# Spockuto/drand

Measured on AMD Instinct MI355X. Metric: beacons verified/s (batch chain verify), higher is better.
Workload: dtype u32 (381-bit Montgomery, 12x32-bit limbs); 1 GPU; configs[1]: 1000000-round chained beacon history per GPU, chain.VerifyBeacon per round; beacons_per_gpu=1000000, segment_len=64, parallelism=range-shard x1

## Files before the change

drand_amd/_lib.py:

```python
from __future__ import annotations

import ctypes
import os

_HERE = os.path.dirname(os.path.abspath(__file__))
LIB_PATH = os.environ.get("DRAND_AMD_LIB", os.path.join(_HERE, "libblsverify.so"))

BLSV_OK = 0
BLSV_EINVAL = -1
BLSV_EHIP = -2
BLSV_ENOGROUP = -3
BLSV_ENOTENOUGH = -4

AGG_OK = 0
AGG_OK_V2 = 1
AGG_V1_RECOVER_FAIL = 2
AGG_V1_INVALID = 3
AGG_V2_RECOVER_FAIL = 4

REJ_OK = 0
REJ_LENGTH = 1
REJ_FLAG = 2
REJ_INF_NONZERO = 3
REJ_X_GE_P = 4
REJ_NOT_ON_CURVE = 5
REJ_NOT_IN_SUBGROUP = 6
REJ_PAIRING = 7
REJ_SHARE_INDEX = 8

REJ_NAMES = {
    REJ_OK: "ok",
    REJ_LENGTH: "bad length",
    REJ_FLAG: "bad compression flag",
    REJ_INF_NONZERO: "infinity with non-zero bits",
    REJ_X_GE_P: "coordinate >= p",
    REJ_NOT_ON_CURVE: "point is not on curve",
    REJ_NOT_IN_SUBGROUP: "point is not on correct subgroup",
    REJ_PAIRING: "bls: invalid signature",
    REJ_SHARE_INDEX: "tbls: invalid signature share",
}

u8p = ctypes.POINTER(ctypes.c_uint8)
u32p = ctypes.POINTER(ctypes.c_uint32)
u64p = ctypes.POINTER(ctypes.c_uint64)
vp = ctypes.c_void_p
sz = ctypes.c_size_t

SIGNATURES = {
    "blsv_version": (ctypes.c_char_p, []),
    "blsv_device_count": (ctypes.c_int, []),
    "blsv_create": (ctypes.c_int, [ctypes.c_int, ctypes.POINTER(vp)]),
    "blsv_destroy": (None, [vp]),
    "blsv_last_error": (ctypes.c_char_p, [vp]),
    "blsv_synchronize": (ctypes.c_int, [vp]),
    "blsv_set_group": (ctypes.c_int, [vp, u8p, sz, sz]),
    "blsv_verify_chained": (ctypes.c_int, [vp, ctypes.c_uint64, u8p, sz, u8p, sz, u8p, u64p, u8p]),
    "blsv_verify_chained_multi": (ctypes.c_int, [ctypes.POINTER(vp), sz, ctypes.POINTER(sz), ctypes.c_uint64, u8p, sz,
                                                  u8p, sz, u8p, u64p, u8p]),
    "blsv_verify_prevs": (ctypes.c_int, [vp, ctypes.c_uint64, u8p, sz, u8p, sz, u8p, u64p, u8p]),
    "blsv_verify_unchained": (ctypes.c_int, [vp, u64p, ctypes.c_uint64, u8p, sz, u8p, u64p, u8p]),
    "blsv_verify_messages": (ctypes.c_int, [vp, u8p, u8p, u32p, sz, u8p, u8p, u64p, u8p]),
    "blsv_verify_partials": (ctypes.c_int, [vp, u8p, sz, u8p, sz, sz, u8p, u8p]),
    "blsv_verify_partials_multi": (ctypes.c_int, [vp, u8p, u32p, u8p, sz, sz, u8p, u8p]),
    "blsv_recover": (ctypes.c_int, [vp, u8p, sz, u8p, sz, sz, sz, sz, u8p]),
    "blsv_aggregate": (ctypes.c_int, [vp, u8p, sz, u8p, sz, sz, sz, sz, u8p, u8p, u8p, u8p]),
    "blsv_aggregate_round": (ctypes.c_int, [vp, u8p, sz, u8p, sz, u8p, sz, u8p, sz, sz, sz, sz, u8p, u8p, u8p, u8p,
                                             ctypes.POINTER(ctypes.c_int32), u8p]),
    "blsv_sign": (ctypes.c_int, [vp, u8p, ctypes.c_int32, u8p, u32p, sz, u8p]),
    "blsv_verify_chained_dev": (ctypes.c_int, [vp, ctypes.c_uint64, ctypes.c_uint64, ctypes.c_uint64, vp, sz, vp, sz,
                                                vp, vp, vp, vp]),
    "blsv_generate_chained_dev": (ctypes.c_int, [vp, u8p, ctypes.c_uint64, ctypes.c_uint64, vp, sz, vp, sz, vp]),
    "blsv_profile_enable": (ctypes.c_int, [vp, ctypes.c_int]),
    "blsv_profile_read": (ctypes.c_int, [vp, ctypes.POINTER(ctypes.c_double), u64p, u64p, ctypes.c_int]),
    "blsv_lat_trace": (ctypes.c_int, [vp, u64p, ctypes.c_int, ctypes.POINTER(ctypes.c_double), ctypes.c_int]),
    "blsv_test_fp_mul": (ctypes.c_int, [vp, u32p, u32p, sz, u32p]),
    "blsv_test_op": (ctypes.c_int, [vp, ctypes.c_char_p, u32p, sz, u32p]),
    "blsv_test_op_info": (ctypes.c_int, [ctypes.c_int, ctypes.POINTER(ctypes.c_char_p), ctypes.POINTER(ctypes.c_int),
                                         ctypes.POINTER(ctypes.c_int), ctypes.POINTER(ctypes.c_int)]),
    "blsv_test_pairing": (ctypes.c_int, [vp, u32p, u32p, sz, u32p]),
    "blsv_test_hash_to_g2": (ctypes.c_int, [vp, u8p, u32p, sz, u32p, u8p]),
    "blsv_test_final_exp": (ctypes.c_int, [vp, u32p, sz, u32p, u32p]),
    "blsv_set_lat_max": (sz, [vp, sz]),
    "blsv_set_chunk": (sz, [vp, sz]),
    "blsv_workspace_bytes": (sz, [vp]),
    "blsv_lat_trace_enable": (ctypes.c_int, [vp, ctypes.c_int]),
    "blsv_test_generic_chains": (ctypes.c_int, [vp, ctypes.c_int]),
    "blsv_test_spec_stats": (ctypes.c_int, [vp, ctypes.POINTER(ctypes.c_uint64), ctypes.POINTER(ctypes.c_uint64)]),
    "blsv_test_lagrange": (ctypes.c_int, [ctypes.POINTER(ctypes.c_uint32), ctypes.c_size_t, ctypes.POINTER(ctypes.c_uint32)]),
    "blsv_service_create": (ctypes.c_int, [ctypes.c_int, ctypes.c_uint32, ctypes.c_uint32, ctypes.POINTER(vp)]),
    "blsv_service_destroy": (None, [vp]),
    "blsv_service_verify_partial": (ctypes.c_int, [vp, u8p, sz, sz, u8p, sz, u8p, sz, u8p, u8p]),
    "blsv_service_verify_recovered": (ctypes.c_int, [vp, u8p, u8p, sz, u8p, u8p, u8p]),
    "blsv_service_stats": (ctypes.c_int, [vp, u64p, u64p, u64p]),
    "blsv_test_service_limits": (ctypes.c_int, [vp, sz, sz, sz, u64p]),
    "blsv_verify_chained_rlc": (ctypes.c_int, [vp, ctypes.c_uint64, u8p, sz, u8p, sz, u8p, u64p, u8p]),
    "blsv_verify_unchained_rlc": (ctypes.c_int, [vp, u64p, ctypes.c_uint64, u8p, sz, u8p, u64p, u8p]),
    "blsv_verify_chained_rlc_dev": (ctypes.c_int, [vp, ctypes.c_uint64, ctypes.c_uint64, ctypes.c_uint64, vp, sz, vp,
                                                    sz, vp, vp, vp, vp]),
    "blsv_set_rlc_group": (sz, [vp, sz]),
    "blsv_rlc_stats": (ctypes.c_int, [vp, u64p, u64p, u64p]),
    "blsv_test_rlc_seed": (ctypes.c_int, [vp, u8p]),
    "blsv_test_rlc_sums": (ctypes.c_int, [vp, ctypes.c_uint64, u8p, sz, u8p, sz, u8p, u8p]),
    "blsv_tlock_open": (ctypes.c_int, [vp, u8p, u8p, sz, u8p, u8p, u8p, u8p]),
    "blsv_tlock_open_dev": (ctypes.c_int, [vp, u8p, vp, sz, vp, vp, vp]),
    "blsv_tlock_stats": (ctypes.c_int, [vp, u64p, u64p]),
}

_lib = None


class EngineUnavailable(RuntimeError):
    """The HIP engine library could not be loaded (no silent fallback exists)."""


def load():
    global _lib
    if _lib is not None:
        return _lib
    if not os.path.exists(LIB_PATH):
        raise EngineUnavailable(
            f"{LIB_PATH} not found: build it with `python -c 'import __graft_entry__ as g; g.build()'` "
            "(make -C drand_amd/csrc); drand_amd has no CPU fallback")
    try:
        lib = ctypes.CDLL(LIB_PATH)
    except OSError as e:
        raise EngineUnavailable(f"cannot load {LIB_PATH}: {e}") from e
    for name, (res, args) in SIGNATURES.items():
        fn = getattr(lib, name)
        fn.restype = res
        fn.argtypes = args
    _lib = lib
    return lib


def buf(data):
    if data is None:
        return None
    b = bytes(data)
    arr = (ctypes.c_uint8 * max(len(b), 1)).from_buffer_copy(b if b else b"\0")
    return arr


def out_buf(n):
    return (ctypes.c_uint8 * max(n, 1))()
```

drand_amd/csrc/blsverify.cpp:

```cpp
#include "host_internal.h"

void release_workspace(blsv_ctx* c) {
  for (DBuf* d : {&c->H, &c->HQ, &c->S, &c->F, &c->FW, &c->LN, &c->h_inf, &c->s_inf, &c->cls}) d->release();
  c->cap = 0;
}

int ensure_workspace(blsv_ctx* c, size_t cnt) {
  for (;;) {
    size_t want = std::min(std::max(cnt, size_t(64)), c->chunk);
    want = (want + 63) & ~size_t(63);
    if (want <= c->cap) return BLSV_OK;
    hipError_t e = hipSuccess;
    auto need = [&](DBuf& d, size_t bytes) {
      if (e == hipSuccess) e = d.ensure(bytes);
    };
    need(c->H, want * blsk::H_WORDS * 4);
    need(c->HQ, want * blsk::HQ_WORDS * 4);
    need(c->S, want * blsk::S_WORDS * 4);
    need(c->F, want * blsk::F_WORDS * 4);
    need(c->FW, 3 * want * blsk::F_WORDS * 4);
    need(c->LN, std::max(std::min(want, kLineSub) * blsk::MILLER_LINE_WORDS, blsk::FEXP_PARK_WORDS(want)) * 4);
    need(c->h_inf, want);
    need(c->s_inf, want);
    need(c->cls, want);
    static_assert(3 * blsk::F_WORDS >= 48 * 64 / 21 + 1, "FW holds the Miller park of a sub-chunk");
    if (e == hipSuccess) {
      c->cap = want;
      return BLSV_OK;
    }
    release_workspace(c);
    (void)hipGetLastError();
    if (e != hipErrorOutOfMemory || want <= kMinChunk)
      return fail(c, BLSV_EHIP, "staging for %zu items: %s", want, hipGetErrorString(e));
    c->chunk = std::max(kMinChunk, ((want / 2) + 63) & ~size_t(63));
    c->lat_max = std::min(c->lat_max, c->chunk);
    c->oom_halvings++;
  }
}

hipError_t h2d(blsv_ctx* c, void* dst, const void* src, size_t len) {
  if (!len) return hipSuccess;
  if (len > kIoCap / 4) return hipMemcpyAsync(dst, src, len, hipMemcpyHostToDevice, c->stream);
  if (!c->io_up.p) {
    hipError_t e = c->io_up.ensure(kIoCap);
    if (e != hipSuccess) return e;
  }
  if (c->io_up_off + len > kIoCap) {
    hipError_t e = hipStreamSynchronize(c->stream);
    if (e != hipSuccess) return e;
    c->io_up_off = 0;
  }
  uint8_t* h = c->io_up.as<uint8_t>() + c->io_up_off;
  memcpy(h, src, len);
  c->io_up_off += (len + 63) & ~size_t(63);
  return hipMemcpyAsync(dst, h, len, hipMemcpyHostToDevice, c->stream);
}

hipError_t download_sync(blsv_ctx* c, std::initializer_list<Down> ds) {
  size_t total = 0;
  for (const Down& d : ds) total += (d.len + 63) & ~size_t(63);
  const bool staged = total <= kIoCap && (c->io_down.p || c->io_down.ensure(kIoCap) == hipSuccess);
  hipError_t e = hipSuccess;
  size_t off = 0;
  for (const Down& d : ds) {
    if (!d.len) continue;
    void* to = staged ? (void*)(c->io_down.as<uint8_t>() + off) : d.user;
    if (e == hipSuccess) e = hipMemcpyAsync(to, d.dev, d.len, hipMemcpyDeviceToHost, c->stream);
    off += (d.len + 63) & ~size_t(63);
  }
  const hipError_t es = hipStreamSynchronize(c->stream);
  if (e == hipSuccess) e = es;
  if (e == hipSuccess) c->io_up_off = 0;
  if (e != hipSuccess || !staged) return e;
  off = 0;
  for (const Down& d : ds) {
    if (d.len) memcpy(d.user, c->io_down.as<uint8_t>() + off, d.len);
    off += (d.len + 63) & ~size_t(63);
  }
  return hipSuccess;
}

hipEvent_t take_event(blsv_ctx* c) {
  if (!c->event_pool.empty()) {
    hipEvent_t e = c->event_pool.back();
    c->event_pool.pop_back();
    return e;
  }
  hipEvent_t e = nullptr;
  if (hipEventCreate(&e) != hipSuccess) return nullptr;
  return e;
}

extern "C" {

const char* blsv_version(void) { return "drand_amd blsverify 0.1 (gfx950)"; }

int blsv_device_count(void) {
  int n = 0;
  return hipGetDeviceCount(&n) == hipSuccess ? n : 0;
}

int blsv_create(int device, blsv_ctx** out) {
  if (!out) return BLSV_EINVAL;
  *out = nullptr;
  blsv_ctx* c = new blsv_ctx();
  c->device = device;
  hipError_t e = hipSetDevice(device);
  if (e == hipSuccess) e = hipStreamCreateWithFlags(&c->stream, hipStreamNonBlocking);
  if (e == hipSuccess) e = hipStreamCreateWithFlags(&c->side, hipStreamNonBlocking);
  if (e == hipSuccess) e = hipStreamCreateWithFlags(&c->side2, hipStreamNonBlocking);
  for (hipEvent_t& ev : c->hash_ev)
    if (e == hipSuccess) e = hipEventCreateWithFlags(&ev, hipEventDisableTiming);
  if (e == hipSuccess) e = hipEventCreateWithFlags(&c->fork_ev, hipEventDisableTiming);
  if (e == hipSuccess) e = hipEventCreateWithFlags(&c->join_ev, hipEventDisableTiming);
  if (e != hipSuccess) {
    fprintf(stderr, "blsv_create: %s\n", hipGetErrorString(e));
    blsv_destroy(c);
    return BLSV_EHIP;
  }
  *out = c;
  return BLSV_OK;
}

void blsv_destroy(blsv_ctx* c) {
  if (!c) return;
  (void)hipSetDevice(c->device);
  for (hipStream_t s : {c->stream, c->side, c->side2}) {
    if (!s) continue;
    (void)hipStreamSynchronize(s);
    (void)hipStreamDestroy(s);
  }
  for (hipEvent_t ev : c->hash_ev)
    if (ev) (void)hipEventDestroy(ev);
  if (c->fork_ev) (void)hipEventDestroy(c->fork_ev);
  if (c->join_ev) (void)hipEventDestroy(c->join_ev);
  (void)hipDeviceSynchronize();
  for (auto& r : c->recs) {
    (void)hipEventDestroy(r.a);
    (void)hipEventDestroy(r.b);
  }
  for (auto e : c->event_pool) (void)hipEventDestroy(e);
  delete c;
}

const char* blsv_last_error(const blsv_ctx* c) { return c ? c->err.c_str() : "null context"; }

int blsv_synchronize(blsv_ctx* c) {
  if (!c) return BLSV_EINVAL;
  HIPCHK(c, hipStreamSynchronize(c->stream));
  return BLSV_OK;
}

int blsv_profile_enable(blsv_ctx* c, int on) {
  if (!c) return BLSV_EINVAL;
  c->prof = on != 0;
  return BLSV_OK;
}

int blsv_profile_read(blsv_ctx* c, double* ms, uint64_t* launches, uint64_t* items, int nstages) {
  if (!c || nstages < 0) return BLSV_EINVAL;
  (void)hipSetDevice(c->device);
  for (int s = 0; s < nstages; s++) {
    if (ms) ms[s] = 0;
    if (launches) launches[s] = 0;
    if (items) items[s] = 0;
  }
  for (auto& r : c->recs) {
    HIPCHK(c, hipEventSynchronize(r.b));
    float t = 0;
    HIPCHK(c, hipEventElapsedTime(&t, r.a, r.b));
    if (r.stage < nstages) {
      if (ms) ms[r.stage] += t;
      if (launches) launches[r.stage] += 1;
      if (items) items[r.stage] += r.items;
    }
    c->event_pool.push_back(r.a);
    c->event_pool.push_back(r.b);
  }
  c->recs.clear();
  return ST_N;
}

size_t blsv_set_lat_max(blsv_ctx* c, size_t lat_max) {
  if (!c) return 0;
  const size_t prev = c->lat_max;
  c->lat_max = std::min(lat_max, c->chunk);
  return prev;
}

size_t blsv_set_chunk(blsv_ctx* c, size_t items) {
  if (!c) return 0;
  const size_t prev = c->chunk;
  size_t v = items ? std::min(std::max(items, kMinChunk), kMaxChunk) : chunk_env();
  v = (v + 63) & ~size_t(63);
  (void)hipSetDevice(c->device);
  if (v < c->cap) {
    (void)hipStreamSynchronize(c->stream);
    (void)hipStreamSynchronize(c->side);
    release_workspace(c);
  }
  c->chunk = v;
  c->lat_max = std::min(c->lat_max, v);
  return prev;
}

size_t blsv_workspace_bytes(const blsv_ctx* c) {
  if (!c) return 0;
  size_t b = 0;
  for (const DBuf* d : {&c->H, &c->HQ, &c->S, &c->F, &c->FW, &c->LN, &c->h_inf, &c->s_inf, &c->cls}) b += d->sz;
  return b;
}

}
```

drand_amd/csrc/engine_ctx.h:

```cpp
#pragma once
#include <hip/hip_runtime.h>

#include <algorithm>
#include <cerrno>
#include <cstdarg>
#include <cstdio>
#include <cstdlib>
#include <cstring>
#include <string>
#include <vector>

#include "../../include/blsverify.h"
#include "kernels.h"

namespace blsv_detail {

constexpr size_t kMaxChunk = size_t(1) << 20;
constexpr size_t kMinChunk = size_t(1) << 14;
constexpr size_t kLineSub = kMaxChunk;
constexpr size_t kPkTable = 4096;
constexpr size_t kStagingBytesPerItem =
    4 * (blsk::H_WORDS + blsk::HQ_WORDS + blsk::S_WORDS + 4 * blsk::F_WORDS + blsk::MILLER_LINE_WORDS) + 3;
static_assert(576ull * kMaxChunk < 0x7fffffffull, "SoA object resource exceeds its 31-bit num_records");
static_assert((133ull * kMaxChunk) * 4 < 0xffffffffull, "SoA VGPR byte offset exceeds 32 bits");
static_assert(48ull * 4 * kMaxChunk < 0x7fffffffull, "3-lane park slot resource exceeds 31 bits");
static_assert(blsk::G1_WORDS <= blsk::H_WORDS, "timelock: the U table does not fit the H staging");
static_assert(blsk::F_WORDS <= blsk::HQ_WORDS, "timelock: the captured Fp12 does not fit the HQ staging");
static_assert(BLSV_GT_LEN == 4 * blsk::F_WORDS, "timelock: the Gt encoding is one F staging row per item");
static_assert(BLSV_U_LEN <= 4 * blsk::S_WORDS, "timelock: a host call's compressed U bytes do not fit the S staging");

struct DBuf {
  void* p = nullptr;
  size_t sz = 0;
  ~DBuf() {
    if (p) (void)hipFree(p);
  }
  void release() {
    if (p) (void)hipFree(p);
    p = nullptr;
    sz = 0;
  }
  hipError_t ensure(size_t need) {
    if (need <= sz) return hipSuccess;
    if (p) {
      (void)hipFree(p);
      p = nullptr;
      sz = 0;
    }
    size_t want = std::max(need, size_t(256));
    hipError_t e = hipMalloc(&p, want);
    if (e == hipSuccess) sz = want;
    return e;
  }
  template <typename T>
  T* as() const {
    return static_cast<T*>(p);
  }
};

struct PinBuf {
  void* p = nullptr;
  size_t sz = 0;
  ~PinBuf() {
    if (p) (void)hipHostFree(p);
  }
  hipError_t ensure(size_t need) {
    if (need <= sz) return hipSuccess;
    if (p) (void)hipHostFree(p);
    p = nullptr;
    sz = 0;
    const size_t want = std::max(need + need / 2, size_t(4096));
    hipError_t e = hipHostMalloc(&p, want, hipHostMallocDefault);
    if (e == hipSuccess) sz = want;
    return e;
  }
  template <typename T>
  T* as() const {
    return static_cast<T*>(p);
  }
};

}
using namespace blsv_detail;

enum Stage {
  ST_HASH = 0,
  ST_DECOMP = 1,
  ST_MILLER = 2,
  ST_FEXP = 3,
  ST_FINISH = 4,
  ST_LAT = 5,
  ST_RLC = 6,
  ST_TLOCK = 7,
  ST_N = 8
};
struct ProfRec {
  int stage;
  size_t items;
  hipEvent_t a, b;
};

constexpr size_t kRlcGroupDefault = 64;
constexpr size_t kRlcGroupMin = 8, kRlcGroupMax = 4096;
constexpr size_t kLatMaxDefault = 1536;
inline size_t chunk_env() {
  static const size_t v = [] {
    const char* e = getenv("BLSV_CHUNK");
    if (!e) return kMaxChunk;
    char* end = nullptr;
    errno = 0;
    const unsigned long long x = strtoull(e, &end, 10);
    if (end == e || *end != '\0' || errno == ERANGE || e[0] == '-' || x == 0) {
      fprintf(stderr, "blsverify: ignoring BLSV_CHUNK=\"%s\" (not a positive integer); chunk stays %zu\n", e, kMaxChunk);
      return kMaxChunk;
    }
    const size_t c = (size_t)std::min<unsigned long long>(std::max<unsigned long long>(x, kMinChunk), kMaxChunk);
    return (c + 63) & ~size_t(63);
  }();
  return v;
}

inline size_t lat_max_env() {
  static const size_t v = [] {
    const char* e = getenv("BLSV_LAT_MAX");
    if (!e) return kLatMaxDefault;
    char* end = nullptr;
    errno = 0;
    const unsigned long long x = strtoull(e, &end, 10);
    if (end == e || *end != '\0' || errno == ERANGE || e[0] == '-') {
      fprintf(stderr, "blsverify: ignoring BLSV_LAT_MAX=\"%s\" (not a non-negative integer); cutover stays %zu\n", e,
              kLatMaxDefault);
      return kLatMaxDefault;
    }
    return (size_t)std::min<unsigned long long>(x, kMaxChunk);
  }();
  return v;
}

struct rlc_state {
  size_t group = kRlcGroupDefault;
  bool seed_pinned = false;
  uint8_t seed[32] = {0};
  uint64_t groups = 0, groups_failed = 0, items_exact = 0;
  DBuf part, gH, gS, g_hinf, g_sinf, gcls, cH, cS, c_hinf, c_sinf, ccls, fail, out96;
  PinBuf host;
};

struct tlock_state {
  bool valid = false;
  uint8_t sig[96] = {0};
  uint8_t cls = 0;
  uint64_t prepared = 0, items = 0;
  DBuf d_sig, S, s_inf, s_cls, tab;
};

struct blsv_ctx {
  int device = 0;
  bool prof = false;
  size_t chunk = chunk_env();
  size_t lat_max = std::min(lat_max_env(), chunk);
  uint64_t oom_halvings = 0;
  std::vector<ProfRec> recs;
  std::vector<hipEvent_t> event_pool;
  hipStream_t stream = nullptr;
  hipStream_t side = nullptr;
  hipEvent_t fork_ev = nullptr, join_ev = nullptr;
  hipStream_t side2 = nullptr;
  hipEvent_t hash_ev[2] = {nullptr, nullptr};
  std::string err;
  bool has_group = false;
  size_t t = 0, n = 0;
  DBuf commits, commit_inf;
  std::vector<uint8_t> group_bytes;
  DBuf pk_all, pk_all_inf;
  size_t pk_all_n = 0;
  bool pk_all_built = false;
  DBuf pk_tab, pk_inf;
  uint8_t pk_cache[48];
  bool pk_cache_valid = false;
  size_t cap = 0;
  DBuf H, S, F, FW, LN, h_inf, s_inf, cls;
  DBuf HQ;
  DBuf in_sigs, in_msgs, in_off, in_len, in_rounds, seeds, bitmap, first_bad, sk, idx, lambdas, scratch, out,
      pp_tab, pp_inf, sel, g1_cls, misc;
  PinBuf pin;
  PinBuf io_up, io_down;
  size_t io_up_off = 0;
  struct SpecSlot {
    DBuf sig, S, s_inf, cls, sel, lam, scratch, out, vmsg, voff, vlen, vcls;
    DBuf hout, saff;
    PinBuf host;
  } spec[2];
  uint64_t spec_hits = 0, spec_misses = 0;
  DBuf arena;
  rlc_state rlc;
  tlock_state tlock;
};

#define HIPCHK(ctx, expr)                                                             \
  do {                                                                                \
    hipError_t e_ = (expr);                                                           \
    if (e_ != hipSuccess) return fail((ctx), BLSV_EHIP, "%s: %s", #expr, hipGetErrorString(e_)); \
  } while (0)

inline int fail(blsv_ctx* ctx, int code, const char* fmt, ...) {
  char buf[512];
  va_list ap;
  va_start(ap, fmt);
  vsnprintf(buf, sizeof buf, fmt, ap);
  va_end(ap);
  if (ctx) ctx->err = buf;
  return code;
}


int ensure_workspace(blsv_ctx* c, size_t cnt);
void release_workspace(blsv_ctx* c);

int svc_verify_mixed(blsv_ctx* c, size_t n, const uint8_t* msgs, const uint64_t* off, const uint32_t* lens,
                     const uint8_t* sigs96, const uint32_t* idx, const uint32_t* d_tab, const uint8_t* d_tab_inf,
                     uint8_t* cls_out);
```

drand_amd/csrc/host_internal.h:

```cpp
#pragma once
#include <functional>
#include <initializer_list>

#include "engine_ctx.h"
#include "hostlogic.h"

#pragma GCC visibility push(hidden)

constexpr size_t kIoCap = size_t(1) << 20;
hipError_t h2d(blsv_ctx* c, void* dst, const void* src, size_t len);
struct Down {
  void* user;
  const void* dev;
  size_t len;
};
hipError_t download_sync(blsv_ctx* c, std::initializer_list<Down> ds);

hipEvent_t take_event(blsv_ctx* c);
struct StageTimer {
  blsv_ctx* c;
  int stage;
  size_t items;
  hipStream_t st;
  hipEvent_t a = nullptr;
  StageTimer(blsv_ctx* c_, int stage_, size_t items_, hipStream_t st_) : c(c_), stage(stage_), items(items_), st(st_) {
    if (c->prof && (a = take_event(c))) (void)hipEventRecord(a, st);
  }
  ~StageTimer() {
    if (!a) return;
    hipEvent_t b = take_event(c);
    if (!b) return;
    (void)hipEventRecord(b, st);
    c->recs.push_back({stage, items, a, b});
  }
};

struct Staging {
  uint32_t *H, *HQ, *S, *F, *FW, *LN;
  uint8_t *h_inf, *s_inf, *cls;
};
inline Staging staging(const blsv_ctx* c) {
  return {c->H.as<uint32_t>(),    c->HQ.as<uint32_t>(),   c->S.as<uint32_t>(),
          c->F.as<uint32_t>(),    c->FW.as<uint32_t>(),   c->LN.as<uint32_t>(),
          c->h_inf.as<uint8_t>(), c->s_inf.as<uint8_t>(), c->cls.as<uint8_t>()};
}

struct SigSrc {
  const uint8_t* d;
  size_t stride, offset;
};
struct PkSel {
  const uint32_t* tab;
  const uint8_t* inf;
  const uint32_t* idx;
};
inline PkSel group_pk(const blsv_ctx* c) { return {c->commits.as<uint32_t>(), c->commit_inf.as<uint8_t>(), nullptr}; }

inline void hash_chained(blsv_ctx* c, const blsk::ChainedSrc& src, size_t base, size_t cnt, hipStream_t st) {
  const Staging w = staging(c);
  blsk::launch_hash_chained(src, base, cnt, w.H, w.h_inf, w.HQ, st);
}
inline void hash_messages(blsv_ctx* c, const uint8_t* d_msgs, const uint64_t* d_off, const uint32_t* d_len, size_t base,
                          size_t cnt, hipStream_t st) {
  const Staging w = staging(c);
  blsk::launch_hash_messages(d_msgs, d_off + base, d_len + base, cnt, w.H, w.h_inf, w.HQ, st);
}
inline void hash_uploaded(blsv_ctx* c, size_t base, size_t cnt, hipStream_t st) {
  hash_messages(c, c->in_msgs.as<uint8_t>(), c->in_off.as<uint64_t>(), c->in_len.as<uint32_t>(), base, cnt, st);
}
inline void lat_uploaded(blsv_ctx* c, const SigSrc& sig, size_t cnt, const PkSel& pk, uint8_t* cls, uint32_t* S,
                         uint8_t* s_inf, hipStream_t st) {
  blsk::launch_lat_messages(c->in_msgs.as<uint8_t>(), c->in_off.as<uint64_t>(), c->in_len.as<uint32_t>(), sig.d,
                            sig.stride, sig.offset, cnt, pk.tab, pk.inf, pk.idx, cls, S, s_inf, st);
}
inline void final_exp(blsv_ctx* c, size_t cnt, uint8_t* cls, hipStream_t st, uint32_t* out = nullptr) {
  const Staging w = staging(c);
  blsk::launch_final_exp(w.F, w.FW, cnt, cls, st, w.LN, out);
}

inline bool use_lat(const blsv_ctx* c, size_t n) { return n > 0 && n <= std::min(c->lat_max, c->cap); }
inline bool use_rlc(const blsv_ctx* c, size_t n) { return n > c->lat_max && n >= 2 * c->rlc.group; }

template <typename F>
inline int for_each_pass(const blsv_ctx* c, size_t n, F f) {
  for (size_t base = 0; base < n; base += c->cap) {
    const int rc = f(base, std::min(c->cap, n - base));
    if (rc) return rc;
  }
  return BLSV_OK;
}

using HashFn = std::function<void(size_t base, size_t cnt, hipStream_t st)>;
struct Tail {
  bool randomized = false;
  uint32_t seed[8] = {0};
  bool fused_subgroup() const { return !randomized; }
};
struct PassOut {
  uint64_t* bitmap;
  unsigned long long* first_bad;
  uint8_t* cls;
  uint64_t label0;
};
int run_head(blsv_ctx* c, const SigSrc& sig, size_t base, size_t cnt, const Tail& tail, hipStream_t st,
             const HashFn& hash);
int run_passes(blsv_ctx* c, size_t n, const SigSrc& sig, const PkSel& pk, const HashFn& hash, const Tail& tail,
               const PassOut& out, hipStream_t st);
int ctx_outputs(blsv_ctx* c, size_t n, bool with_cls, PassOut& out);

int rlc_draw_seed(blsv_ctx* c, uint32_t (&w)[8]);
int rlc_sums(blsv_ctx* c, size_t base, size_t cnt, const uint32_t (&seed)[8], hipStream_t st);

int stage_chain(blsv_ctx* c, uint64_t first_round, const uint8_t* prevs, size_t prev0_len, bool prev_rows,
                const uint8_t* sigs96, size_t n, blsk::ChainedSrc& src);
int decode_g1(blsv_ctx* c, const uint8_t* pk48, size_t cnt, DBuf& tab, DBuf& inf, std::vector<uint8_t>& cls);
int upload_messages(blsv_ctx* c, const uint8_t* msgs, const uint32_t* msg_lens, size_t n);

#pragma GCC visibility pop
```

drand_amd/csrc/hostlogic.h:

```cpp
#pragma once
#include <stddef.h>
#include <stdint.h>

#include <algorithm>
#include <vector>

#include "../../include/blsverify.h"

#pragma GCC visibility push(hidden)
namespace blsv_detail {

inline void scalar_mod_r(const uint8_t* be32, uint32_t out[8]) {
  static const uint32_t R[8] = {0x00000001u, 0xffffffffu, 0xfffe5bfeu, 0x53bda402u,
                                0x09a1d805u, 0x3339d808u, 0x299d7d48u, 0x73eda753u};
  for (int i = 0; i < 8; i++) {
    const uint8_t* q = be32 + 28 - 4 * i;
    out[i] = ((uint32_t)q[0] << 24) | ((uint32_t)q[1] << 16) | ((uint32_t)q[2] << 8) | q[3];
  }
  for (int rep = 0; rep < 4; rep++) {
    bool ge = true;
    for (int i = 7; i >= 0; i--) {
      if (out[i] != R[i]) {
        ge = out[i] > R[i];
        break;
      }
    }
    if (!ge) break;
    uint64_t br = 0;
    for (int i = 0; i < 8; i++) {
      uint64_t d = (uint64_t)out[i] - R[i] - br;
      out[i] = (uint32_t)d;
      br = (d >> 63) & 1;
    }
  }
}

namespace hfr {
typedef unsigned __int128 u128;
static const uint64_t RM[4] = {0xffffffff00000001ull, 0x53bda402fffe5bfeull, 0x3339d80809a1d805ull,
                               0x73eda753299d7d48ull};
struct E {
  uint64_t l[4];
};
inline bool geq_r(const uint64_t (&a)[5]) {
  if (a[4]) return true;
  for (int i = 3; i >= 0; i--)
    if (a[i] != RM[i]) return a[i] > RM[i];
  return true;
}
inline void sub_r(uint64_t (&a)[5]) {
  uint64_t br = 0;
  for (int i = 0; i < 4; i++) {
    const u128 d = (u128)a[i] - RM[i] - br;
    a[i] = (uint64_t)d;
    br = (uint64_t)(d >> 64) & 1u;
  }
  a[4] -= br;
}
inline uint64_t n0() {
  uint64_t inv = 1;
  for (int k = 0; k < 7; k++) inv *= 2 - RM[0] * inv;
  return (uint64_t)0 - inv;
}
inline E mul(const E& a, const E& b) {
  static const uint64_t N0 = n0();
  uint64_t t[6] = {0, 0, 0, 0, 0, 0};
  for (int i = 0; i < 4; i++) {
    uint64_t c = 0;
    for (int j = 0; j < 4; j++) {
      const u128 v = (u128)a.l[j] * b.l[i] + t[j] + c;
      t[j] = (uint64_t)v;
      c = (uint64_t)(v >> 64);
    }
    u128 v = (u128)t[4] + c;
    t[4] = (uint64_t)v;
    t[5] = (uint64_t)(v >> 64);
    const uint64_t m = t[0] * N0;
    v = (u128)m * RM[0] + t[0];
    c = (uint64_t)(v >> 64);
    for (int j = 1; j < 4; j++) {
      v = (u128)m * RM[j] + t[j] + c;
      t[j - 1] = (uint64_t)v;
      c = (uint64_t)(v >> 64);
    }
    v = (u128)t[4] + c;
    t[3] = (uint64_t)v;
    t[4] = t[5] + (uint64_t)(v >> 64);
  }
  uint64_t r[5] = {t[0], t[1], t[2], t[3], t[4]};
  if (geq_r(r)) sub_r(r);
  return {{r[0], r[1], r[2], r[3]}};
}
inline E add(const E& a, const E& b) {
  uint64_t r[5];
  uint64_t c = 0;
  for (int i = 0; i < 4; i++) {
    const u128 v = (u128)a.l[i] + b.l[i] + c;
    r[i] = (uint64_t)v;
    c = (uint64_t)(v >> 64);
  }
  r[4] = c;
  if (geq_r(r)) sub_r(r);
  return {{r[0], r[1], r[2], r[3]}};
}
inline const E& r2() {
  static const E v = [] {
    E x = {{1, 0, 0, 0}};
    for (int k = 0; k < 512; k++) x = add(x, x);
    return x;
  }();
  return v;
}
inline E from_int(int64_t v) {
  E x = {{(uint64_t)(v < 0 ? -v : v), 0, 0, 0}};
  if (v < 0) {
    uint64_t a[5] = {RM[0], RM[1], RM[2], RM[3], 0};
    uint64_t br = 0;
    for (int i = 0; i < 4; i++) {
      const u128 d = (u128)a[i] - x.l[i] - br;
      a[i] = (uint64_t)d;
      br = (uint64_t)(d >> 64) & 1u;
    }
    x = {{a[0], a[1], a[2], a[3]}};
  }
  return mul(x, r2());
}
inline E inv(const E& a) {
  uint64_t e[4] = {RM[0] - 2, RM[1], RM[2], RM[3]};
  E acc = from_int(1);
  for (int i = 255; i >= 0; i--) {
    acc = mul(acc, acc);
    if ((e[i >> 6] >> (i & 63)) & 1u) acc = mul(acc, a);
  }
  return acc;
}
}

inline void host_lagrange(const uint32_t* idx, size_t t, uint32_t* out) {
  std::vector<hfr::E> num(t), den(t), pre(t + 1);
  for (size_t i = 0; i < t; i++) {
    const int64_t xi = (int64_t)idx[i] + 1;
    hfr::E n = hfr::from_int(1), d = n;
    for (size_t j = 0; j < t; j++) {
      if (j == i) continue;
      const int64_t xj = (int64_t)idx[j] + 1;
      n = hfr::mul(n, hfr::from_int(xj));
      d = hfr::mul(d, hfr::from_int(xj - xi));
    }
    num[i] = n;
    den[i] = d;
  }
  pre[0] = hfr::from_int(1);
  for (size_t i = 0; i < t; i++) pre[i + 1] = hfr::mul(pre[i], den[i]);
  hfr::E run = hfr::inv(pre[t]);
  const hfr::E one_plain = {{1, 0, 0, 0}};
  for (size_t i = t; i-- > 0;) {
    const hfr::E di = hfr::mul(run, pre[i]);
    run = hfr::mul(run, den[i]);
    const hfr::E lam = hfr::mul(hfr::mul(num[i], di), one_plain);
    for (int w = 0; w < 4; w++) {
      out[i * 8 + 2 * w] = (uint32_t)lam.l[w];
      out[i * 8 + 2 * w + 1] = (uint32_t)(lam.l[w] >> 32);
    }
  }
}

inline void bitmap_words_to_bytes(const uint64_t* w, size_t n, uint8_t* out) {
  for (size_t i = 0; i < (n + 7) / 8; i++) {
    uint8_t b = (uint8_t)(w[i / 8] >> (8 * (i % 8)));
    if (i == (n + 7) / 8 - 1 && (n % 8)) b &= (uint8_t)((1u << (n % 8)) - 1);
    out[i] = b;
  }
}

inline uint64_t fold_classes(const uint8_t* cls, size_t n, uint8_t* ok_bitmap) {
  uint64_t fb = UINT64_MAX;
  for (size_t i = 0; i < n; i++) {
    if (cls[i] != BLSV_REJ_OK && fb == UINT64_MAX) fb = i;
    if (ok_bitmap) {
      if (i % 8 == 0) ok_bitmap[i / 8] = 0;
      ok_bitmap[i / 8] |= (uint8_t)((cls[i] == BLSV_REJ_OK) << (i % 8));
    }
  }
  return fb;
}

inline void or_bits_at(uint8_t* dst, const uint8_t* src, size_t cnt, size_t pos) {
  const size_t nb = (cnt + 7) / 8, q = pos / 8, s = pos % 8;
  for (size_t j = 0; j < nb; j++) {
    uint8_t b = src[j];
    if (j == nb - 1 && (cnt % 8)) b &= (uint8_t)((1u << (cnt % 8)) - 1);
    dst[q + j] |= (uint8_t)(b << s);
    if (s && (b >> (8 - s))) dst[q + j + 1] |= (uint8_t)(b >> (8 - s));
  }
}

inline void share_indices(const uint8_t* partials, size_t partial_len, size_t k, std::vector<uint32_t>& index) {
  index.assign(k, 0);
  if (partial_len < 2) return;
  for (size_t i = 0; i < k; i++) index[i] = ((uint32_t)partials[i * partial_len] << 8) | partials[i * partial_len + 1];
}

inline bool select_shares(const std::vector<uint8_t>& cls, const std::vector<uint32_t>& index, size_t lo, size_t hi,
                          size_t t, size_t n, std::vector<uint32_t>& sel, std::vector<uint32_t>& idx) {
  sel.clear();
  idx.clear();
  size_t taken = 0;
  for (size_t i = lo; i < hi && taken < t; i++) {
    if (cls[i] != BLSV_REJ_OK) continue;
    taken++;
    if (index[i] >= n || std::find(idx.begin(), idx.end(), index[i]) != idx.end()) continue;
    sel.push_back((uint32_t)i);
    idx.push_back(index[i]);
  }
  return sel.size() >= t;
}

inline size_t rlc_failing_items(size_t cnt, size_t G, const uint32_t* fail, size_t nf) {
  const size_t ng = (cnt + G - 1) / G;
  return nf * G - (fail[nf - 1] == ng - 1 ? ng * G - cnt : 0);
}

struct SvcLayout {
  size_t o_len, o_idx, o_sig, o_msg, total;
};
inline SvcLayout svc_layout(size_t n, size_t mbytes) {
  SvcLayout l;
  l.o_len = (n + 1) * 8;
  l.o_idx = l.o_len + ((n * 4 + 7) & ~size_t(7));
  l.o_sig = l.o_idx + ((n * 4 + 7) & ~size_t(7));
  l.o_msg = l.o_sig + n * 96;
  l.total = l.o_msg + mbytes + 8;
  return l;
}

}
#pragma GCC visibility pop
```

drand_amd/csrc/k_fexp.hip:

```cpp
#include "kcommon.h"

namespace blsk {

BLS_KERNEL(BLS_WPE_FEXP) k_fexp_easy(const uint32_t* F, size_t cnt, const uint8_t* cls, uint32_t* G) {
  size_t i = (size_t)blockIdx.x * TPB + threadIdx.x;
  if (i >= cnt || cls[i] != REJ_OK) return;
  st_fp12(G, cnt, i, fexp_easy(ld_fp12(F, cnt, i)));
}

#ifndef BLS_WPE_FEXP_TRI
#define BLS_WPE_FEXP_TRI 2
#endif

struct TriPark {
  uint32_t* p;
  size_t n, i;
};

template <typename LoadX>
DI fp4 tri_pow_x_abs(const tri_lane& t, LoadX lx, const TriPark& pk) {
  constexpr uint64_t NSQ = 1ull | (2ull << 6) | (3ull << 12) | (9ull << 18) | (32ull << 24) | (16ull << 30);
  fp4 r = lx();
#pragma unroll 1
  for (int s = 0; s < 6; s++) {
    const int n = (int)((NSQ >> (6 * s)) & 63u);
#pragma unroll 1
    for (int k = 0; k < n; k++) r = tri_cyclotomic_sqr(t, r);
    if (s < 5) r = tri_mul_lp(t, r, lx(), pk.p, pk.n, pk.i);
  }
  return r;
}

template <int MODE>
BLS_KERNEL(BLS_WPE_FEXP_TRI) k_fexp_tri(const uint32_t* X, const uint32_t* C, const uint32_t* G, size_t cnt,
                                        uint8_t* cls, uint32_t* OUT, uint32_t* park) {
  const tri_lane t = tri_lane_id();
#if BLS_CSQR_LIN
  kp_lds_init<11>();
#endif
  const size_t ir = (size_t)blockIdx.x * TRI_GROUPS + t.group;
  const bool in_range = t.group < TRI_GROUPS && ir < cnt;
  const size_t i0 = in_range ? ir : cnt - 1;
  const bool live = in_range && cls[i0] == REJ_OK;
  const TriPark pk = {park, (size_t)gridDim.x * TPB, (size_t)blockIdx.x * TPB + t.lane};
  auto at = [&](const uint32_t* B) {
    size_t j = i0;
    asm volatile("" : "+v"(j));
    return tri_load(B, cnt, j, t.role);
  };
  fp4 r = tri_conj(t, tri_pow_x_abs(t, [&]() { return at(X); }, pk));
  if (MODE == 0 || MODE == 1) r = tri_mul_lp(t, r, tri_conj(t, at(X)), pk.p, pk.n, pk.i);
  if (MODE == 2) r = tri_mul_lp(t, r, tri_frob(t, at(X)), pk.p, pk.n, pk.i);
  if (MODE == 4) {
    r = tri_mul_lp(t, r, tri_frob2(t, at(C)), pk.p, pk.n, pk.i);
    r = tri_mul_lp(t, r, tri_conj(t, at(C)), pk.p, pk.n, pk.i);
    r = tri_mul_lp(t, r, tri_cyclotomic_sqr(t, at(G)), pk.p, pk.n, pk.i);
    r = tri_mul_lp(t, r, at(G), pk.p, pk.n, pk.i);
  }
  if (MODE < 4 || OUT) {
    if (live) tri_store(OUT, cnt, i0, t.role, r);
  }
  if (MODE == 4) {
    const bool one = tri_is_one(t, r);
    if (live && t.role == 0 && !one) cls[i0] = REJ_PAIRING;
  }
}

void launch_final_exp(uint32_t* F, uint32_t* W, size_t cnt, uint8_t* cls, hipStream_t st, uint32_t* park,
                      uint32_t* out) {
  if (!cnt) return;
  uint32_t* G = W;
  uint32_t* B = W + cnt * F_WORDS;
  uint32_t* C = W + 2 * cnt * F_WORDS;
  const dim3 grid(grid_for(cnt)), blk(TPB);
  hipLaunchKernelGGL(k_fexp_easy, grid, blk, 0, st, F, cnt, cls, G);
  const dim3 tgrid((unsigned)((cnt + TRI_GROUPS - 1) / TRI_GROUPS));
  hipLaunchKernelGGL(k_fexp_tri<0>, tgrid, blk, 0, st, G, nullptr, nullptr, cnt, cls, F, park);
  hipLaunchKernelGGL(k_fexp_tri<1>, tgrid, blk, 0, st, F, nullptr, nullptr, cnt, cls, B, park);
  hipLaunchKernelGGL(k_fexp_tri<2>, tgrid, blk, 0, st, B, nullptr, nullptr, cnt, cls, C, park);
  hipLaunchKernelGGL(k_fexp_tri<3>, tgrid, blk, 0, st, C, nullptr, nullptr, cnt, cls, F, park);
  hipLaunchKernelGGL(k_fexp_tri<4>, tgrid, blk, 0, st, F, C, G, cnt, cls, out, park);
}

}
```

drand_amd/csrc/k_miller.hip:

```cpp
#include <type_traits>

#include "kcommon.h"
#include "testops.h"

namespace blsk {

DI int line_slot(int step, int k) { return (step * 2 + k) * 6; }
#ifndef BLS_LN_AUX
#define BLS_LN_AUX 2
#endif
#ifndef BLS_LN_AUX_ST
#define BLS_LN_AUX_ST BLS_LN_AUX
#endif
#ifndef BLS_LN_AUX_LD
#define BLS_LN_AUX_LD BLS_LN_AUX
#endif

static __shared__ uint32_t g_ml_T[72 * BLS_LANES];
struct g2proj_lds {
  uint32_t* base;
  DI fp2 get(int c) const {
    fp2 v;
#pragma unroll
    for (int w = 0; w < 12; w++) {
      v.c0.l[w] = base[(24 * c + w) * BLS_LANES];
      v.c1.l[w] = base[(24 * c + 12 + w) * BLS_LANES];
    }
    return v;
  }
  DI void set(int c, const fp2& v) const {
#pragma unroll
    for (int w = 0; w < 12; w++) {
      base[(24 * c + w) * BLS_LANES] = v.c0.l[w];
      base[(24 * c + 12 + w) * BLS_LANES] = v.c1.l[w];
    }
  }
};

template <bool CHECK>
BLS_KERNEL(BLS_WPE_LINES)
k_miller_lines(const uint32_t* pk_tab, const uint8_t* pk_inf, const uint32_t* pk_idx, const uint32_t* H,
               const uint8_t* h_inf, const uint32_t* S, const uint8_t* s_inf,
               std::conditional_t<CHECK, uint8_t*, const uint8_t*> cls, size_t cnt, size_t base, size_t m, size_t sub,
               uint32_t* LN) {
  const int k = (int)(blockIdx.x & 1u);
  const size_t i = (size_t)(blockIdx.x >> 1) * TPB + threadIdx.x;
  if (i >= m) return;
  const size_t g = base + i;
  if (cls[g] != REJ_OK) return;
  const uint32_t kk = pk_idx ? pk_idx[g] : 0u;
  const bool act[2] = {!(pk_inf[kk] | h_inf[g]), !s_inf[g]};
  {
    const uint32_t* Qb = k == 0 ? H : S;
    auto load_q = [&]() {
      size_t j = g;
      asm volatile("" : "+v"(j));
      return g2a{ld_fp2(Qb, cnt, j, 0), ld_fp2(Qb, cnt, j, 2)};
    };
    auto emit = [&](int step, const line& l) {
      const int s = line_slot(step, k);
      const line o = act[k] ? l : line_one();
      st_fp2<BLS_LN_AUX_ST>(LN, sub, i, s + 0, o.a0);
      st_fp2<BLS_LN_AUX_ST>(LN, sub, i, s + 2, o.a1);
      st_fp2<BLS_LN_AUX_ST>(LN, sub, i, s + 4, o.a4);
    };
    auto pcoord = [&](int c) {
      size_t o = (size_t)kk * G1_WORDS + 12 * c;
      asm volatile("" : "+v"(o));
      fp v;
#pragma unroll
      for (int w = 0; w < 12; w++) v.l[w] = pk_tab[o + w];
      return k == 0 ? v : fp_load_const(c == 0 ? G1_GEN_X : G1_GEN_NEG_Y);
    };
    if (!act[k]) {
#pragma unroll 1
      for (int s = 0; s < MILLER_STEPS; s++) emit(s, line_one());
      return;
    }
    int step = 0;
    auto put = [&](int c, const fp2& v) { st_fp2<BLS_LN_AUX_ST>(LN, sub, i, line_slot(step, k) + 2 * c, v); };
    auto xp = [&]() { return pcoord(0); };
    auto yp = [&]() { return pcoord(1); };
    const g2proj_lds T{g_ml_T + threadIdx.x};
    {
      const g2a Q0 = load_q();
      T.set(0, Q0.x);
      T.set(1, Q0.y);
      T.set(2, fp2_one());
    }
#pragma unroll 1
    for (int b = 62; b >= 0; b--) {
      miller_dbl_step_ts(T, put, xp, yp);
      step++;
      if ((BLS_X_ABS >> b) & 1ull) {
        miller_add_step_ts(T, load_q, put, xp, yp);
        step++;
      }
    }
    if constexpr (CHECK) {
      if (k == 1 && !miller_t_in_subgroup(T, load_q)) {
        size_t j = g;
        asm volatile("" : "+v"(j));
        cls[j] = REJ_NOT_IN_SUBGROUP;
      }
    }
  }
}

static __shared__ uint32_t g_mf_L[120 * BLS_LANES];
DI void mf_put(int c, const fp2& v) {
  const unsigned l = threadIdx.x;
#pragma unroll
  for (int k = 0; k < 12; k++) {
    g_mf_L[(c * 24 + k) * BLS_LANES + l] = v.c0.l[k];
    g_mf_L[(c * 24 + 12 + k) * BLS_LANES + l] = v.c1.l[k];
  }
}
DI fp2 mf_get(int c) {
  unsigned l = threadIdx.x;
  asm volatile("" : "+v"(l));
  fp2 v;
#pragma unroll
  for (int k = 0; k < 12; k++) {
    v.c0.l[k] = g_mf_L[(c * 24 + k) * BLS_LANES + l];
    v.c1.l[k] = g_mf_L[(c * 24 + 12 + k) * BLS_LANES + l];
  }
  return v;
}
using KpLds16 = KpLdsK<16>;

template <typename LB>
DI fp6 fp6_mul_lb(const fp6& a, LB lb) {
#if BLS_F6_LIN
  return fp6_mul_lin_lb(a, lb, KpLds16());
#else
  fp2 t0 = fp2_mul(a.c0, lb(0));
  fp2 t1 = fp2_mul(a.c1, lb(1));
  fp2 t2 = fp2_mul(a.c2, lb(2));
  fp2 c0 = fp2_add(fp2_mul_xi(fp2_sub(fp2_sub(fp2_mul(fp2_add_lazy(a.c1, a.c2), fp2_add_lazy(lb(1), lb(2))), t1), t2)), t0);
  fp2 c1 = fp2_add(fp2_sub(fp2_sub(fp2_mul(fp2_add_lazy(a.c0, a.c1), fp2_add_lazy(lb(0), lb(1))), t0), t1), fp2_mul_xi(t2));
  fp2 c2 = fp2_add(fp2_sub(fp2_sub(fp2_mul(fp2_add_lazy(a.c0, a.c2), fp2_add_lazy(lb(0), lb(2))), t0), t2), t1);
  return {c0, c1, c2};
#endif
}
DI fp12 fp12_mul_by_line_pair_lds(const fp12& f) {
  const fp6 t0 = fp6_mul_lb(f.c0, [](int c) { return mf_get(c); });
  fp6 t1;
  {
    const fp2 b1 = mf_get(3), b2 = mf_get(4);
    t1 = fp6_mul_by_12(f.c1, b1, b2);
  }
  const fp6 c1 = fp6_sub(fp6_sub(fp6_mul_lb(fp6_add_lazy(f.c0, f.c1), [](int c) {
                                   return c == 0 ? mf_get(0) : fp2_add_lazy(mf_get(c), mf_get(c + 2));
                                 }),
                                 t0),
                         t1);
  return {fp6_add(t0, fp6_mul_v(t1)), c1};
}

BLS_KERNEL(BLS_WPE_MILLER_F) k_miller_f(const uint32_t* LN, const uint8_t* cls, size_t cnt, size_t base,
                                                  size_t m, size_t sub, uint32_t* F) {
#if BLS_F6_LIN
  kp_lds_init<16>();
#endif
  const size_t i = (size_t)blockIdx.x * TPB + threadIdx.x;
  if (i >= m) return;
  const size_t g = base + i;
  if (cls[g] != REJ_OK) return;
  auto load = [&](int step, int k) {
    const int s = line_slot(step, k);
    return line{ld_fp2<BLS_LN_AUX_LD>(LN, sub, i, s + 0), ld_fp2<BLS_LN_AUX_LD>(LN, sub, i, s + 2),
                ld_fp2<BLS_LN_AUX_LD>(LN, sub, i, s + 4)};
  };
  fp12 f = fp12_one();
  int step = 0;
#pragma unroll 1
  for (int b = 62; b >= 0; b--) {
#pragma unroll 1
    for (int rep = 0; rep < 2; rep++) {
      if (rep == 1 && !((BLS_X_ABS >> b) & 1ull)) break;
#if BLS_F6_LIN
      if (rep == 0 && b != 62) f = fp12_sqr_lin(f, KpLds16());
#else
      if (rep == 0 && b != 62) f = fp12_sqr(f);
#endif
      {
        const fp12 L = line_mul_line(load(step, 0), load(step, 1));
        if (step == 0) {
          f = L;
          step++;
          continue;
        }
        mf_put(0, L.c0.c0);
        mf_put(1, L.c0.c1);
        mf_put(2, L.c0.c2);
        mf_put(3, L.c1.c1);
        mf_put(4, L.c1.c2);
      }
      f = fp12_mul_by_line_pair_lds(f);
      step++;
    }
  }
  st_fp12(F, cnt, g, fp12_conj(f));
}

constexpr uint64_t miller_sq_bits(int half) {
  uint64_t m = 0;
  int s = 0;
  for (int i = 62; i >= 0; i--) {
    if (i != 62 && s / 64 == half) m |= 1ull << (s % 64);
    s++;
    if ((BLS_X_ABS >> i) & 1ull) s++;
  }
  return m;
}
constexpr uint64_t MILLER_SQ_LO = miller_sq_bits(0), MILLER_SQ_HI = miller_sq_bits(1);

#ifndef BLS_MILLER_TRI_MAX
#define BLS_MILLER_TRI_MAX 65536
#endif
constexpr size_t kMillerTriMax = BLS_MILLER_TRI_MAX;

#ifndef BLS_WPE_MILLER_TRI
#define BLS_WPE_MILLER_TRI 2
#endif

BLS_KERNEL(BLS_WPE_MILLER_TRI) k_miller_f_tri(const uint32_t* LN, const uint8_t* cls, size_t cnt, size_t base,
                                              size_t m, size_t sub, uint32_t* F, uint32_t* park) {
  const tri_lane t = tri_lane_id();
  const size_t ir = (size_t)blockIdx.x * TRI_GROUPS + t.group;
  const bool in_range = t.group < TRI_GROUPS && ir < m;
  const size_t i = in_range ? ir : m - 1;
  const bool live = in_range && cls[base + i] == REJ_OK;
  const size_t park_n = (size_t)gridDim.x * TPB, park_i = (size_t)blockIdx.x * TPB + t.lane;
  fp4 A;
#pragma unroll 1
  for (int s = 0; s < MILLER_STEPS; s++) {
    const bool sq = ((s < 64 ? MILLER_SQ_LO >> s : MILLER_SQ_HI >> (s - 64)) & 1ull) != 0;
    if (sq) A = tri_sqr_lp(t, A);
    const int s0 = line_slot(s, 0), s1 = line_slot(s, 1);
    auto la = [&](int c) {
      size_t j = i;
      asm volatile("" : "+v"(j));
      return ld_fp2_v<BLS_LN_AUX_LD>(LN + (size_t)s0 * 12 * sub, sub, j, 2 * c);
    };
    auto lb = [&](int c) {
      size_t j = i;
      asm volatile("" : "+v"(j));
      return ld_fp2_v<BLS_LN_AUX_LD>(LN + (size_t)s1 * 12 * sub, sub, j, 2 * c);
    };
    const fp4 L = tri_line_pair(t, la, lb);
    if (s == 0) {
      A = L;
    } else {
      A = tri_mul_lp(t, A, L, park, park_n, park_i);
    }
  }
  A = tri_conj(t, A);
  if (live) tri_store(F, cnt, base + i, t.role, A);
}

template <int OP, int NIN, int NOUT>
__global__ void __launch_bounds__(TPB) k_test_op_mf(const uint32_t* in, size_t cnt, uint32_t* out) {
#if BLS_F6_LIN
  kp_lds_init<16>();
#endif
  const size_t i = (size_t)blockIdx.x * TPB + threadIdx.x;
  if (i >= cnt) return;
  fp x[NIN], r[NOUT];
#pragma unroll
  for (int k = 0; k < NIN; k++)
#pragma unroll
    for (int w = 0; w < 12; w++) x[k].l[w] = in[(i * NIN + k) * 12 + w];
  if constexpr (OP == TOP_fp6_mul_lb) {
#pragma unroll
    for (int c = 0; c < 3; c++) mf_put(c, t_f2(x, 6 + 2 * c));
    t_put6(r, 0, fp6_mul_lb(t_f6(x, 0), [](int c) { return mf_get(c); }));
  } else {
#pragma unroll
    for (int c = 0; c < 5; c++) mf_put(c, t_f2(x, 12 + 2 * c));
    t_put12(r, 0, fp12_mul_by_line_pair_lds(t_f12(x, 0)));
  }
#pragma unroll
  for (int k = 0; k < NOUT; k++)
#pragma unroll
    for (int w = 0; w < 12; w++) out[(i * NOUT + k) * 12 + w] = r[k].l[w];
}

bool launch_test_op_mf(int op, const uint32_t* in, size_t cnt, uint32_t* out, hipStream_t st) {
  if (op != TOP_fp6_mul_lb && op != TOP_fp12_mul_by_line_pair_lds) return false;
  if (!cnt) return true;
  if (op == TOP_fp6_mul_lb)
    hipLaunchKernelGGL((k_test_op_mf<TOP_fp6_mul_lb, 12, 6>), dim3(grid_for(cnt)), dim3(TPB), 0, st, in, cnt, out);
  else
    hipLaunchKernelGGL((k_test_op_mf<TOP_fp12_mul_by_line_pair_lds, 22, 12>), dim3(grid_for(cnt)), dim3(TPB), 0, st, in,
                       cnt, out);
  return true;
}

void launch_miller(const uint32_t* pk_tab, const uint8_t* pk_inf, const uint32_t* pk_idx, const uint32_t* H,
                   const uint8_t* h_inf, const uint32_t* S, const uint8_t* s_inf, uint8_t* cls, size_t cnt,
                   uint32_t* F, uint32_t* LN, size_t sub, uint32_t* park, bool check_subgroup, hipStream_t st) {
  if (!cnt) return;
  for (size_t b = 0; b < cnt; b += sub) {
    const size_t m = cnt - b < sub ? cnt - b : sub;
    if (check_subgroup)
      hipLaunchKernelGGL(k_miller_lines<true>, dim3(2 * grid_for(m)), dim3(TPB), 0, st, pk_tab, pk_inf, pk_idx, H,
                         h_inf, S, s_inf, cls, cnt, b, m, sub, LN);
    else
      hipLaunchKernelGGL(k_miller_lines<false>, dim3(2 * grid_for(m)), dim3(TPB), 0, st, pk_tab, pk_inf, pk_idx, H,
                         h_inf, S, s_inf, (const uint8_t*)cls, cnt, b, m, sub, LN);
    if (m <= kMillerTriMax) {
      hipLaunchKernelGGL(k_miller_f_tri, dim3((unsigned)((m + TRI_GROUPS - 1) / TRI_GROUPS)), dim3(TPB), 0, st, LN,
                         cls, cnt, b, m, sub, F, park);
    } else {
      hipLaunchKernelGGL(k_miller_f, dim3(grid_for(m)), dim3(TPB), 0, st, LN, cls, cnt, b, m, sub, F);
    }
  }
}

}
```

drand_amd/csrc/kernels.h:

```cpp
#pragma once
#include <hip/hip_runtime.h>
#include <stddef.h>
#include <stdint.h>

namespace blsk {

constexpr int H_WORDS = 48;
constexpr int S_WORDS = 48;
constexpr int F_WORDS = 144;
constexpr int G1_WORDS = 24;

struct ChainedSrc {
  const uint8_t* sigs;
  const uint8_t* seeds;
  uint64_t first_round;
  uint64_t seg_len;
  uint32_t seed0_len;
  uint64_t seg_phase;
};

constexpr int HQ_WORDS = 144;
void launch_hash_chained(const ChainedSrc& src, size_t base, size_t cnt, uint32_t* H, uint8_t* h_inf,
                         uint32_t* Q, hipStream_t st);
void launch_hash_unchained(const uint64_t* rounds, uint64_t first_round, size_t base, size_t cnt, uint32_t* H,
                           uint8_t* h_inf, uint32_t* Q, hipStream_t st);
void launch_hash_messages(const uint8_t* msgs, const uint64_t* off, const uint32_t* len, size_t cnt,
                          uint32_t* H, uint8_t* h_inf, uint32_t* Q, hipStream_t st);
void launch_decompress_g2(const uint8_t* sigs, size_t stride, size_t offset, size_t base, size_t cnt, uint32_t* S,
                          uint8_t* s_inf, uint8_t* cls, hipStream_t st);
constexpr int MILLER_LINE_WORDS = 68 * 2 * 6 * 12;
void launch_miller(const uint32_t* pk_tab, const uint8_t* pk_inf, const uint32_t* pk_idx, const uint32_t* H,
                   const uint8_t* h_inf, const uint32_t* S, const uint8_t* s_inf, uint8_t* cls, size_t cnt,
                   uint32_t* F, uint32_t* LN, size_t sub, uint32_t* park, bool check_subgroup, hipStream_t st);
constexpr size_t TRI_PARK_WORDS(size_t items) { return 48 * 64 * ((items + 20) / 21); }
constexpr size_t FEXP_PARK_WORDS(size_t items) { return TRI_PARK_WORDS(items); }
void launch_final_exp(uint32_t* F, uint32_t* W, size_t cnt, uint8_t* cls, hipStream_t st, uint32_t* park,
                      uint32_t* out = nullptr);
void launch_finish(const uint8_t* cls, size_t base, size_t cnt, uint64_t* bitmap, unsigned long long* first_bad,
                   uint64_t label0, hipStream_t st);

constexpr size_t kRlcLaneItems = 8;
constexpr size_t kRlcPartWords = 72;
constexpr size_t rlc_lanes(size_t cnt) { return (cnt + kRlcLaneItems - 1) / kRlcLaneItems; }
constexpr size_t rlc_groups(size_t cnt, size_t group) { return (cnt + group - 1) / group; }
void launch_rlc_sums(const uint32_t* H, const uint8_t* h_inf, const uint32_t* S, const uint8_t* s_inf,
                     const uint8_t* cls, size_t cnt, uint64_t index0, const uint32_t* seed_words, size_t group,
                     uint32_t* part, uint32_t* GH, uint8_t* g_hinf, uint32_t* GS, uint8_t* g_sinf, hipStream_t st);
void launch_rlc_gather(const uint32_t* fail, size_t group, size_t m, const uint32_t* H, const uint8_t* h_inf,
                       const uint32_t* S, const uint8_t* s_inf, const uint8_t* cls, size_t cnt, uint32_t* CH,
                       uint8_t* c_hinf, uint32_t* CS, uint8_t* c_sinf, uint8_t* ccls, hipStream_t st);
void launch_rlc_scatter(const uint32_t* fail, size_t group, size_t m, const uint8_t* ccls, uint8_t* cls, size_t cnt,
                        hipStream_t st);
void launch_rlc_compress(const uint32_t* GP, const uint8_t* g_inf, size_t ng, uint8_t* out96, hipStream_t st);

constexpr size_t kTlockTabWords = 68 * 3 * 24;
void launch_tlock_prepare(const uint32_t* S, const uint8_t* s_inf, const uint8_t* s_cls, uint32_t* tab, hipStream_t st);
void launch_tlock_f(const uint32_t* tab, const uint32_t* U, const uint8_t* u_inf, const uint8_t* cls,
                    const uint8_t* sig_inf, size_t cnt, uint32_t* F, hipStream_t st);
void launch_tlock_encode(const uint32_t* E, const uint8_t* cls, size_t cnt, uint8_t* out, hipStream_t st);

int lat_trace_read(uint64_t* out, int n, hipStream_t st);
int lat_trace_clear(hipStream_t st);
int lat_trace_enable(int on, hipStream_t st);
extern int g_generic_chains_all;
void launch_lat_chained(const ChainedSrc& src, size_t base, size_t cnt, const uint32_t* pk_tab, const uint8_t* pk_inf,
                        uint8_t* cls, hipStream_t st);
void launch_lat_unchained(const uint64_t* rounds, uint64_t first_round, const uint8_t* sigs, size_t base, size_t cnt,
                          const uint32_t* pk_tab, const uint8_t* pk_inf, uint8_t* cls, hipStream_t st);
void launch_lat_messages(const uint8_t* msgs, const uint64_t* off, const uint32_t* len, const uint8_t* sigs,
                         size_t stride, size_t offset, size_t cnt, const uint32_t* pk_tab, const uint8_t* pk_inf,
                         const uint32_t* pk_idx, uint8_t* cls, uint32_t* S, uint8_t* s_inf, hipStream_t st);

void launch_decompress_g1(const uint8_t* in, size_t cnt, uint32_t* tab, uint8_t* inf, uint8_t* cls, hipStream_t st);
void launch_pubpoly_eval(const uint32_t* commits, const uint8_t* commit_inf, uint32_t t, const uint32_t* idx,
                         size_t cnt, uint32_t* out_tab, uint8_t* out_inf, hipStream_t st);
void launch_lat_decode(const uint8_t* sigs, size_t stride, size_t offset, size_t cnt, uint32_t* S, uint8_t* s_inf,
                       uint8_t* cls, hipStream_t st);
void launch_decompress_g2_only(const uint8_t* sigs, size_t stride, size_t offset, size_t base, size_t cnt,
                               uint32_t* S, uint8_t* s_inf, uint8_t* cls, hipStream_t st);
void launch_lat_recover(const uint32_t* S, size_t n_s, const uint8_t* s_inf, const uint32_t* sel,
                        const uint32_t* lambdas, uint32_t t, uint32_t* scratch, uint8_t* out96, hipStream_t st,
                        uint32_t* saff = nullptr);
constexpr size_t kLatHoutWords = 448, kLatSaffWords = 192;
void launch_lat_hash_key(const uint8_t* msgs, const uint64_t* off, const uint32_t* len, const uint32_t* pk_tab,
                         const uint8_t* pk_inf, uint32_t* hout, hipStream_t st);
void launch_lat_verify_pre(const uint32_t* hout, const uint32_t* saff, uint8_t* cls, hipStream_t st);
void launch_sign(const uint32_t* sk_words, int32_t index, const uint32_t* H, const uint8_t* h_inf, size_t cnt,
                 uint8_t* out, size_t out_stride, hipStream_t st);
void launch_gen_chained(const uint32_t* sk_words, const ChainedSrc& src, size_t n, uint8_t* sigs_out, hipStream_t st);

bool launch_test_op(int op, const uint32_t* in, size_t cnt, uint32_t* out, uint32_t* park, hipStream_t st);
bool launch_test_op_mf(int op, const uint32_t* in, size_t cnt, uint32_t* out, hipStream_t st);
void launch_test_fp_mul(const uint32_t* a, const uint32_t* b, size_t cnt, uint32_t* out, hipStream_t st);
void launch_test_pairing(const uint32_t* p_tab, const uint32_t* q_aff, size_t cnt, uint32_t* out_f, hipStream_t st);
void launch_test_unpack_g2(const uint32_t* H, size_t cnt, uint32_t* out, hipStream_t st);
void launch_test_pack_fp12(const uint32_t* f, size_t cnt, uint32_t* F, hipStream_t st);
void launch_test_unpack_fp12(const uint32_t* F, size_t cnt, uint32_t* out, hipStream_t st);
void launch_test_final_exp_ref(const uint32_t* F, size_t cnt, uint32_t* out, hipStream_t st);

}
```

drand_amd/csrc/testhooks.cpp:

```cpp
#include "../../include/blsverify_testing.h"
#include "host_internal.h"
#include "testops_list.h"

static const bls::TestOpInfo* find_test_op(const char* name, int* op) {
  if (!name) return nullptr;
  const bls::TestOpInfo* tab = bls::test_op_table();
  for (int k = 0; k < bls::TOP_COUNT; k++)
    if (!strcmp(tab[k].name, name)) {
      if (op) *op = k;
      return &tab[k];
    }
  return nullptr;
}

extern "C" {

int blsv_test_lagrange(const uint32_t* idx, size_t t, uint32_t* out) {
  if (!idx || !out) return BLSV_EINVAL;
  for (size_t i = 0; i < t; i++)
    for (size_t j = 0; j < i; j++)
      if (idx[i] == idx[j]) return BLSV_EINVAL;
  host_lagrange(idx, t, out);
  return BLSV_OK;
}

int blsv_test_rlc_seed(blsv_ctx* c, const uint8_t* seed32) {
  if (!c) return BLSV_EINVAL;
  c->rlc.seed_pinned = seed32 != nullptr;
  if (seed32) memcpy(c->rlc.seed, seed32, 32);
  return BLSV_OK;
}

int blsv_test_rlc_sums(blsv_ctx* c, uint64_t first_round, const uint8_t* prev0, size_t prev0_len,
                       const uint8_t* sigs96, size_t n, uint8_t* out_a96, uint8_t* out_b96) {
  if (!c) return BLSV_EINVAL;
  if (!n || !sigs96 || !prev0 || !out_a96 || !out_b96 || (prev0_len != 32 && prev0_len != 96))
    return fail(c, BLSV_EINVAL, "test_rlc_sums: bad arguments");
  (void)hipSetDevice(c->device);
  Tail tail;
  tail.randomized = true;
  int rc = rlc_draw_seed(c, tail.seed);
  if (rc) return rc;
  rc = ensure_workspace(c, n);
  if (rc) return rc;
  blsk::ChainedSrc src;
  rc = stage_chain(c, first_round, prev0, prev0_len, false, sigs96, n, src);
  if (rc) return rc;
  rlc_state& r = c->rlc;
  size_t done = 0;
  rc = for_each_pass(c, n, [&](size_t base, size_t cnt) {
    const size_t ng = blsk::rlc_groups(cnt, r.group);
    int prc = run_head(c, {src.sigs, 96, 0}, base, cnt, tail, c->stream,
                       [&](size_t b, size_t m, hipStream_t st) { hash_chained(c, src, b, m, st); });
    if (prc) return prc;
    prc = rlc_sums(c, base, cnt, tail.seed, c->stream);
    if (prc) return prc;
    HIPCHK(c, r.out96.ensure(2 * ng * 96));
    uint8_t* d_out = r.out96.as<uint8_t>();
    blsk::launch_rlc_compress(r.gH.as<uint32_t>(), r.g_hinf.as<uint8_t>(), ng, d_out, c->stream);
    blsk::launch_rlc_compress(r.gS.as<uint32_t>(), r.g_sinf.as<uint8_t>(), ng, d_out + ng * 96, c->stream);
    HIPCHK(c, hipGetLastError());
    HIPCHK(c, hipMemcpyAsync(out_a96 + done * 96, d_out, ng * 96, hipMemcpyDeviceToHost, c->stream));
    HIPCHK(c, hipMemcpyAsync(out_b96 + done * 96, d_out + ng * 96, ng * 96, hipMemcpyDeviceToHost, c->stream));
    HIPCHK(c, hipStreamSynchronize(c->stream));
    c->io_up_off = 0;
    done += ng;
    return BLSV_OK;
  });
  return rc ? rc : (int)done;
}

int blsv_test_spec_stats(blsv_ctx* c, uint64_t* hits, uint64_t* misses) {
  if (!c || !hits || !misses) return BLSV_EINVAL;
  *hits = c->spec_hits;
  *misses = c->spec_misses;
  return BLSV_OK;
}

int blsv_test_generic_chains(blsv_ctx* c, int on) {
  if (!c) return BLSV_EINVAL;
  blsk::g_generic_chains_all = on != 0;
  return BLSV_OK;
}

int blsv_lat_trace_enable(blsv_ctx* c, int on) {
  if (!c) return BLSV_EINVAL;
  (void)hipSetDevice(c->device);
  if (blsk::lat_trace_enable(on, c->stream) != 0) return fail(c, BLSV_EHIP, "lat_trace_enable: symbol copy failed");
  return BLSV_OK;
}

int blsv_lat_trace(blsv_ctx* c, uint64_t* ticks, int n, double* ticks_per_us, int clear) {
  if (!c || n < 0 || (n && !ticks)) return BLSV_EINVAL;
  (void)hipSetDevice(c->device);
  HIPCHK(c, hipDeviceSynchronize());
  int got = 0;
  if (n) {
    got = blsk::lat_trace_read(ticks, n, c->stream);
    if (got < 0) return fail(c, BLSV_EHIP, "lat_trace: symbol copy failed");
  }
  if (ticks_per_us) {
    int khz = 0;
    HIPCHK(c, hipDeviceGetAttribute(&khz, hipDeviceAttributeWallClockRate, c->device));
    *ticks_per_us = khz / 1000.0;
  }
  if (clear && blsk::lat_trace_clear(c->stream) != 0) return fail(c, BLSV_EHIP, "lat_trace: clear failed");
  HIPCHK(c, hipStreamSynchronize(c->stream));
  return got;
}

int blsv_test_fp_mul(blsv_ctx* c, const uint32_t* a, const uint32_t* b, size_t n, uint32_t* out) {
  if (!c || (n && (!a || !b || !out))) return BLSV_EINVAL;
  (void)hipSetDevice(c->device);
  DBuf da, db, dout;
  HIPCHK(c, da.ensure(n * 48));
  HIPCHK(c, db.ensure(n * 48));
  HIPCHK(c, dout.ensure(n * 48));
  HIPCHK(c, hipMemcpyAsync(da.p, a, n * 48, hipMemcpyHostToDevice, c->stream));
  HIPCHK(c, hipMemcpyAsync(db.p, b, n * 48, hipMemcpyHostToDevice, c->stream));
  blsk::launch_test_fp_mul(da.as<uint32_t>(), db.as<uint32_t>(), n, dout.as<uint32_t>(), c->stream);
  HIPCHK(c, hipGetLastError());
  HIPCHK(c, hipMemcpyAsync(out, dout.p, n * 48, hipMemcpyDeviceToHost, c->stream));
  HIPCHK(c, hipStreamSynchronize(c->stream));
  return BLSV_OK;
}

int blsv_test_pairing(blsv_ctx* c, const uint32_t* p, const uint32_t* q, size_t n, uint32_t* out_f) {
  if (!c || (n && (!p || !q || !out_f))) return BLSV_EINVAL;
  (void)hipSetDevice(c->device);
  DBuf dp, dq, dout;
  HIPCHK(c, dp.ensure(n * 96));
  HIPCHK(c, dq.ensure(n * 192));
  HIPCHK(c, dout.ensure(n * 576));
  HIPCHK(c, hipMemcpyAsync(dp.p, p, n * 96, hipMemcpyHostToDevice, c->stream));
  HIPCHK(c, hipMemcpyAsync(dq.p, q, n * 192, hipMemcpyHostToDevice, c->stream));
  blsk::launch_test_pairing(dp.as<uint32_t>(), dq.as<uint32_t>(), n, dout.as<uint32_t>(), c->stream);
  HIPCHK(c, hipGetLastError());
  HIPCHK(c, hipMemcpyAsync(out_f, dout.p, n * 576, hipMemcpyDeviceToHost, c->stream));
  HIPCHK(c, hipStreamSynchronize(c->stream));
  return BLSV_OK;
}

int blsv_test_final_exp(blsv_ctx* c, const uint32_t* f, size_t n, uint32_t* out_pipeline, uint32_t* out_ref) {
  if (!c || (n && (!f || !out_pipeline || !out_ref))) return BLSV_EINVAL;
  if (n > kMaxChunk) return BLSV_EINVAL;
  (void)hipSetDevice(c->device);
  int rc = ensure_workspace(c, n);
  if (rc) return rc;
  if (n > c->cap) return fail(c, BLSV_EINVAL, "test_final_exp: more than the context chunk");
  if (!n) return BLSV_OK;
  DBuf din, dout, dref;
  HIPCHK(c, din.ensure(n * 576));
  HIPCHK(c, dout.ensure(n * 576));
  HIPCHK(c, dref.ensure(n * 576));
  const Staging w = staging(c);
  HIPCHK(c, hipMemcpyAsync(din.p, f, n * 576, hipMemcpyHostToDevice, c->stream));
  HIPCHK(c, hipMemsetAsync(w.cls, 0, n, c->stream));
  blsk::launch_test_pack_fp12(din.as<uint32_t>(), n, w.F, c->stream);
  blsk::launch_test_final_exp_ref(w.F, n, dref.as<uint32_t>(), c->stream);
  final_exp(c, n, w.cls, c->stream, dout.as<uint32_t>());
  blsk::launch_test_unpack_fp12(dout.as<uint32_t>(), n, din.as<uint32_t>(), c->stream);
  HIPCHK(c, hipMemcpyAsync(out_pipeline, din.p, n * 576, hipMemcpyDeviceToHost, c->stream));
  blsk::launch_test_unpack_fp12(dref.as<uint32_t>(), n, dout.as<uint32_t>(), c->stream);
  HIPCHK(c, hipMemcpyAsync(out_ref, dout.p, n * 576, hipMemcpyDeviceToHost, c->stream));
  HIPCHK(c, hipGetLastError());
  HIPCHK(c, hipStreamSynchronize(c->stream));
  return BLSV_OK;
}

int blsv_test_op_info(int index, const char** name, int* in_fp, int* out_fp, int* lanes) {
  if (index < 0 || index >= bls::TOP_COUNT) return BLSV_EINVAL;
  const bls::TestOpInfo& t = bls::test_op_table()[index];
  if (name) *name = t.name;
  if (in_fp) *in_fp = t.nin;
  if (out_fp) *out_fp = t.nout;
  if (lanes) *lanes = t.kind == 3 ? 3 : 1;
  return BLSV_OK;
}

int blsv_test_op(blsv_ctx* c, const char* name, const uint32_t* in, size_t n, uint32_t* out) {
  int op = 0;
  const bls::TestOpInfo* t = find_test_op(name, &op);
  if (!c || !t || (n && (!in || !out))) return BLSV_EINVAL;
  if (n > kMaxChunk) return BLSV_EINVAL;
  if (!n) return BLSV_OK;
  (void)hipSetDevice(c->device);
  const size_t in_bytes = n * (size_t)t->nin * 48, out_bytes = n * (size_t)t->nout * 48;
  DBuf din, dout, dpark;
  HIPCHK(c, din.ensure(in_bytes));
  HIPCHK(c, dout.ensure(out_bytes));
  if (t->kind == 3) HIPCHK(c, dpark.ensure(blsk::TRI_PARK_WORDS(n) * 4));
  HIPCHK(c, hipMemcpyAsync(din.p, in, in_bytes, hipMemcpyHostToDevice, c->stream));
  HIPCHK(c, hipMemsetAsync(dout.p, 0xA5, out_bytes, c->stream));
  const bool ran = t->kind == 2
                       ? blsk::launch_test_op_mf(op, din.as<uint32_t>(), n, dout.as<uint32_t>(), c->stream)
                       : blsk::launch_test_op(op, din.as<uint32_t>(), n, dout.as<uint32_t>(),
                                              t->kind == 3 ? dpark.as<uint32_t>() : nullptr, c->stream);
  if (!ran) return fail(c, BLSV_EINVAL, "test_op: no kernel for this op");
  HIPCHK(c, hipGetLastError());
  HIPCHK(c, hipMemcpyAsync(out, dout.p, out_bytes, hipMemcpyDeviceToHost, c->stream));
  HIPCHK(c, hipStreamSynchronize(c->stream));
  return BLSV_OK;
}

int blsv_test_hash_to_g2(blsv_ctx* c, const uint8_t* msgs, const uint32_t* msg_lens, size_t n, uint32_t* out,
                         uint8_t* inf) {
  if (!c || (n && (!msg_lens || !out || !inf))) return BLSV_EINVAL;
  if (n > kMaxChunk) return BLSV_EINVAL;
  (void)hipSetDevice(c->device);
  int rc = ensure_workspace(c, n);
  if (rc) return rc;
  if (n > c->cap) return fail(c, BLSV_EINVAL, "test_hash_to_g2: more than the context chunk");
  rc = upload_messages(c, msgs, msg_lens, n);
  if (rc) return rc;
  DBuf dout;
  HIPCHK(c, dout.ensure(n * 192));
  hash_uploaded(c, 0, n, c->stream);
  blsk::launch_test_unpack_g2(c->H.as<uint32_t>(), n, dout.as<uint32_t>(), c->stream);
  HIPCHK(c, hipGetLastError());
  HIPCHK(c, hipMemcpyAsync(out, dout.p, n * 192, hipMemcpyDeviceToHost, c->stream));
  HIPCHK(c, hipMemcpyAsync(inf, c->h_inf.p, n, hipMemcpyDeviceToHost, c->stream));
  HIPCHK(c, hipStreamSynchronize(c->stream));
  return BLSV_OK;
}

}
```

drand_amd/csrc/tlock.cpp:

```cpp
#include "host_internal.h"

static int tlock_prepare_sig(blsv_ctx* c, const uint8_t* sig96, hipStream_t st, uint8_t* sig_class) {
  tlock_state& t = c->tlock;
  if (!t.valid || memcmp(t.sig, sig96, 96) != 0) {
    t.valid = false;
    HIPCHK(c, t.d_sig.ensure(96));
    HIPCHK(c, t.S.ensure(blsk::S_WORDS * 4));
    HIPCHK(c, t.s_inf.ensure(1));
    HIPCHK(c, t.s_cls.ensure(1));
    HIPCHK(c, t.tab.ensure(blsk::kTlockTabWords * 4));
    HIPCHK(c, hipMemcpyAsync(t.d_sig.p, sig96, 96, hipMemcpyHostToDevice, st));
    {
      StageTimer tm(c, ST_TLOCK, 1, st);
      blsk::launch_decompress_g2(t.d_sig.as<uint8_t>(), 96, 0, 0, 1, t.S.as<uint32_t>(), t.s_inf.as<uint8_t>(),
                                 t.s_cls.as<uint8_t>(), st);
      blsk::launch_tlock_prepare(t.S.as<uint32_t>(), t.s_inf.as<uint8_t>(), t.s_cls.as<uint8_t>(),
                                 t.tab.as<uint32_t>(), st);
    }
    HIPCHK(c, hipGetLastError());
    uint8_t cls = 0xff;
    HIPCHK(c, hipMemcpyAsync(&cls, t.s_cls.p, 1, hipMemcpyDeviceToHost, st));
    HIPCHK(c, hipStreamSynchronize(st));
    memcpy(t.sig, sig96, 96);
    t.cls = cls;
    t.valid = true;
    if (cls == BLSV_REJ_OK) t.prepared++;
  }
  if (sig_class) *sig_class = t.cls;
  if (t.cls != BLSV_REJ_OK) return fail(c, BLSV_EINVAL, "tlock_open: signature rejected (class %d)", (int)t.cls);
  return BLSV_OK;
}

static int tlock_pass(blsv_ctx* c, const uint8_t* d_us, size_t cnt, uint8_t* d_out, uint8_t* d_cls_out,
                      hipStream_t st) {
  const tlock_state& t = c->tlock;
  const Staging w = staging(c);
  uint32_t* U = w.H;
  uint8_t* u_inf = w.h_inf;
  uint8_t* ucls = w.s_inf;
  {
    StageTimer tm(c, ST_DECOMP, cnt, st);
    blsk::launch_decompress_g1(d_us, cnt, U, u_inf, ucls, st);
  }
  HIPCHK(c, hipMemcpyAsync(w.cls, ucls, cnt, hipMemcpyDeviceToDevice, st));
  {
    StageTimer tm(c, ST_TLOCK, cnt, st);
    blsk::launch_tlock_f(t.tab.as<uint32_t>(), U, u_inf, ucls, t.s_inf.as<uint8_t>(), cnt, w.F, st);
  }
  {
    StageTimer tm(c, ST_FEXP, cnt, st);
    final_exp(c, cnt, w.cls, st, w.HQ);
  }
  blsk::launch_tlock_encode(w.HQ, ucls, cnt, d_out, st);
  if (d_cls_out) HIPCHK(c, hipMemcpyAsync(d_cls_out, ucls, cnt, hipMemcpyDeviceToDevice, st));
  HIPCHK(c, hipGetLastError());
  return BLSV_OK;
}

static int tlock_passes(blsv_ctx* c, bool host, const uint8_t* us, size_t n, uint8_t* out, uint8_t* cls,
                        hipStream_t st) {
  int rc = ensure_workspace(c, n);
  if (rc) return rc;
  for (size_t base = 0; base < n; base += c->cap) {
    const size_t cnt = std::min(c->cap, n - base);
    const uint8_t* pass_us = us + base * BLSV_U_LEN;
    uint8_t* pass_out = out + base * BLSV_GT_LEN;
    if (host) {
      HIPCHK(c, h2d(c, c->S.p, pass_us, cnt * BLSV_U_LEN));
      rc = tlock_pass(c, c->S.as<uint8_t>(), cnt, c->F.as<uint8_t>(), nullptr, st);
      if (rc) return rc;
      HIPCHK(c, download_sync(c, {{pass_out, c->F.p, cnt * BLSV_GT_LEN}, {cls + base, c->s_inf.p, cnt}}));
    } else {
      rc = tlock_pass(c, pass_us, cnt, pass_out, cls ? cls + base : nullptr, st);
      if (rc) return rc;
    }
  }
  c->tlock.items += n;
  return BLSV_OK;
}

extern "C" {

int blsv_tlock_open(blsv_ctx* c, const uint8_t* sig96, const uint8_t* us48, size_t n, uint8_t* out_gt576, uint8_t* ok,
                    uint8_t* reject_class, uint8_t* sig_class) {
  if (!c) return BLSV_EINVAL;
  if (!sig96 || (n && (!us48 || !out_gt576 || !ok))) return fail(c, BLSV_EINVAL, "tlock_open: bad arguments");
  (void)hipSetDevice(c->device);
  int rc = tlock_prepare_sig(c, sig96, c->stream, sig_class);
  if (rc) return rc;
  if (!n) return BLSV_OK;
  std::vector<uint8_t> own;
  uint8_t* cls = reject_class;
  if (!cls) {
    own.resize(n);
    cls = own.data();
  }
  rc = tlock_passes(c, true, us48, n, out_gt576, cls, c->stream);
  if (rc) return rc;
  for (size_t i = 0; i < n; i++) ok[i] = cls[i] == BLSV_REJ_OK;
  return BLSV_OK;
}

int blsv_tlock_open_dev(blsv_ctx* c, const uint8_t* sig96, const uint8_t* d_us48, size_t n, uint8_t* d_out_gt576,
                        uint8_t* d_reject_class, void* stream) {
  if (!c) return BLSV_EINVAL;
  if (!sig96 || (n && (!d_us48 || !d_out_gt576)) || ((uintptr_t)d_out_gt576 & 3))
    return fail(c, BLSV_EINVAL, "tlock_open_dev: bad arguments");
  (void)hipSetDevice(c->device);
  hipStream_t st = stream ? (hipStream_t)stream : c->stream;
  int rc = tlock_prepare_sig(c, sig96, st, nullptr);
  if (rc) return rc;
  if (!n) return BLSV_OK;
  return tlock_passes(c, false, d_us48, n, d_out_gt576, d_reject_class, st);
}

int blsv_tlock_stats(blsv_ctx* c, uint64_t* prepared, uint64_t* items) {
  if (!c) return BLSV_EINVAL;
  if (prepared) *prepared = c->tlock.prepared;
  if (items) *items = c->tlock.items;
  return BLSV_OK;
}

}
```

drand_amd/csrc/verify.cpp:

```cpp
#include <sys/random.h>

#include <thread>

#include "host_internal.h"

static bool serial_stages() {
  static const bool on = [] {
    const char* e = getenv("BLSV_SERIAL_STAGES");
    return e && e[0] == '1';
  }();
  return on;
}

static void head_decompress(blsv_ctx* c, const SigSrc& sig, size_t base, size_t cnt, const Tail& tail, hipStream_t st) {
  const Staging w = staging(c);
  if (tail.fused_subgroup() && !blsk::g_generic_chains_all)
    blsk::launch_decompress_g2_only(sig.d, sig.stride, sig.offset, base, cnt, w.S, w.s_inf, w.cls, st);
  else
    blsk::launch_decompress_g2(sig.d, sig.stride, sig.offset, base, cnt, w.S, w.s_inf, w.cls, st);
}

int run_head(blsv_ctx* c, const SigSrc& sig, size_t base, size_t cnt, const Tail& tail, hipStream_t st,
             const HashFn& hash) {
  if (serial_stages()) {
    {
      StageTimer tm(c, ST_DECOMP, cnt, st);
      head_decompress(c, sig, base, cnt, tail, st);
    }
    StageTimer tm(c, ST_HASH, cnt, st);
    hash(base, cnt, st);
    return BLSV_OK;
  }
  HIPCHK(c, hipEventRecord(c->fork_ev, st));
  HIPCHK(c, hipStreamWaitEvent(c->side, c->fork_ev, 0));
  {
    StageTimer tm(c, ST_DECOMP, cnt, c->side);
    head_decompress(c, sig, base, cnt, tail, c->side);
  }
  HIPCHK(c, hipEventRecord(c->join_ev, c->side));
  {
    StageTimer tm(c, ST_HASH, cnt, st);
    hash(base, cnt, st);
  }
  HIPCHK(c, hipStreamWaitEvent(st, c->join_ev, 0));
  return BLSV_OK;
}

static void pairing_check(blsv_ctx* c, const PkSel& pk, const uint32_t* H, const uint8_t* h_inf, const uint32_t* S,
                          const uint8_t* s_inf, uint8_t* cls, size_t cnt, bool check_subgroup, hipStream_t st) {
  const Staging w = staging(c);
  {
    StageTimer tm(c, ST_MILLER, cnt, st);
    blsk::launch_miller(pk.tab, pk.inf, pk.idx, H, h_inf, S, s_inf, cls, cnt, w.F, w.LN, std::min(cnt, kLineSub), w.FW,
                        check_subgroup, st);
  }
  StageTimer tm(c, ST_FEXP, cnt, st);
  final_exp(c, cnt, cls, st);
}

static int finish_pass(blsv_ctx* c, size_t base, size_t cnt, const PassOut& out, hipStream_t st) {
  {
    StageTimer tm(c, ST_FINISH, cnt, st);
    blsk::launch_finish(c->cls.as<uint8_t>(), base, cnt, out.bitmap, out.first_bad, out.label0, st);
  }
  if (out.cls) HIPCHK(c, hipMemcpyAsync(out.cls + base, c->cls.p, cnt, hipMemcpyDeviceToDevice, st));
  HIPCHK(c, hipGetLastError());
  return BLSV_OK;
}

static int run_tail(blsv_ctx* c, size_t base, size_t cnt, const PkSel& pk, const PassOut& out, hipStream_t st) {
  const Staging w = staging(c);
  pairing_check(c, pk, w.H, w.h_inf, w.S, w.s_inf, w.cls, cnt, true, st);
  return finish_pass(c, base, cnt, out, st);
}


int rlc_draw_seed(blsv_ctx* c, uint32_t (&w)[8]) {
  uint8_t s[32];
  if (c->rlc.seed_pinned) {
    memcpy(s, c->rlc.seed, 32);
  } else {
    size_t got = 0;
    while (got < sizeof s) {
      const ssize_t r = getrandom(s + got, sizeof s - got, 0);
      if (r < 0 && errno == EINTR) continue;
      if (r <= 0) return fail(c, BLSV_EHIP, "rlc: getrandom failed: %s", strerror(errno));
      got += (size_t)r;
    }
  }
  for (int k = 0; k < 8; k++)
    w[k] = ((uint32_t)s[4 * k] << 24) | ((uint32_t)s[4 * k + 1] << 16) | ((uint32_t)s[4 * k + 2] << 8) | s[4 * k + 3];
  return BLSV_OK;
}

static size_t round64(size_t v) { return (std::max(v, size_t(1)) + 63) & ~size_t(63); }

int rlc_sums(blsv_ctx* c, size_t base, size_t cnt, const uint32_t (&seed)[8], hipStream_t st) {
  rlc_state& r = c->rlc;
  const Staging w = staging(c);
  const size_t ng = blsk::rlc_groups(cnt, r.group), cap = round64(ng);
  HIPCHK(c, r.part.ensure(2 * blsk::kRlcPartWords * blsk::rlc_lanes(cnt) * 4));
  HIPCHK(c, r.gH.ensure(cap * blsk::H_WORDS * 4));
  HIPCHK(c, r.gS.ensure(cap * blsk::S_WORDS * 4));
  HIPCHK(c, r.g_hinf.ensure(cap));
  HIPCHK(c, r.g_sinf.ensure(cap));
  HIPCHK(c, r.gcls.ensure(cap));
  StageTimer tm(c, ST_RLC, cnt, st);
  blsk::launch_rlc_sums(w.H, w.h_inf, w.S, w.s_inf, w.cls, cnt, base, seed, r.group, r.part.as<uint32_t>(),
                        r.gH.as<uint32_t>(), r.g_hinf.as<uint8_t>(), r.gS.as<uint32_t>(), r.g_sinf.as<uint8_t>(), st);
  return BLSV_OK;
}

static int run_tail_rlc(blsv_ctx* c, size_t base, size_t cnt, const uint32_t (&seed)[8], const PassOut& out,
                        hipStream_t st) {
  rlc_state& r = c->rlc;
  const Staging w = staging(c);
  const PkSel pk = group_pk(c);
  const size_t G = r.group, ng = blsk::rlc_groups(cnt, G);
  int rc = rlc_sums(c, base, cnt, seed, st);
  if (rc) return rc;
  HIPCHK(c, hipMemsetAsync(r.gcls.p, 0, ng, st));
  pairing_check(c, pk, r.gH.as<uint32_t>(), r.g_hinf.as<uint8_t>(), r.gS.as<uint32_t>(), r.g_sinf.as<uint8_t>(),
                r.gcls.as<uint8_t>(), ng, false, st);
  HIPCHK(c, hipGetLastError());
  HIPCHK(c, r.host.ensure(kMaxChunk / kRlcGroupMin * 5 + 16));
  uint8_t* verdict = r.host.as<uint8_t>();
  HIPCHK(c, hipMemcpyAsync(verdict, r.gcls.p, ng, hipMemcpyDeviceToHost, st));
  HIPCHK(c, hipStreamSynchronize(st));
  uint32_t* fail_list = reinterpret_cast<uint32_t*>(verdict + ((ng + 7) & ~size_t(7)));
  size_t nf = 0;
  for (size_t g = 0; g < ng; g++)
    if (verdict[g] != BLSV_REJ_OK) fail_list[nf++] = (uint32_t)g;
  r.groups += ng;
  r.groups_failed += nf;
  if (nf) {
    const size_t m = rlc_failing_items(cnt, G, fail_list, nf), cap = round64(m);
    r.items_exact += m;
    HIPCHK(c, r.fail.ensure(nf * 4));
    HIPCHK(c, r.cH.ensure(cap * blsk::H_WORDS * 4));
    HIPCHK(c, r.cS.ensure(cap * blsk::S_WORDS * 4));
    HIPCHK(c, r.c_hinf.ensure(cap));
    HIPCHK(c, r.c_sinf.ensure(cap));
    HIPCHK(c, r.ccls.ensure(cap));
    HIPCHK(c, hipMemcpyAsync(r.fail.p, fail_list, nf * 4, hipMemcpyHostToDevice, st));
    {
      StageTimer tm(c, ST_RLC, m, st);
      blsk::launch_rlc_gather(r.fail.as<uint32_t>(), G, m, w.H, w.h_inf, w.S, w.s_inf, w.cls, cnt, r.cH.as<uint32_t>(),
                              r.c_hinf.as<uint8_t>(), r.cS.as<uint32_t>(), r.c_sinf.as<uint8_t>(), r.ccls.as<uint8_t>(),
                              st);
    }
    pairing_check(c, pk, r.cH.as<uint32_t>(), r.c_hinf.as<uint8_t>(), r.cS.as<uint32_t>(), r.c_sinf.as<uint8_t>(),
                  r.ccls.as<uint8_t>(), m, false, st);
    StageTimer tm(c, ST_RLC, m, st);
    blsk::launch_rlc_scatter(r.fail.as<uint32_t>(), G, m, r.ccls.as<uint8_t>(), w.cls, cnt, st);
  }
  return finish_pass(c, base, cnt, out, st);
}

int run_passes(blsv_ctx* c, size_t n, const SigSrc& sig, const PkSel& pk, const HashFn& hash, const Tail& tail,
               const PassOut& out, hipStream_t st) {
  return for_each_pass(c, n, [&](size_t base, size_t cnt) {
    const PkSel pass_pk{pk.tab, pk.inf, pk.idx ? pk.idx + base : nullptr};
    const int rc = run_head(c, sig, base, cnt, tail, st, hash);
    if (rc) return rc;
    return tail.randomized ? run_tail_rlc(c, base, cnt, tail.seed, out, st) : run_tail(c, base, cnt, pass_pk, out, st);
  });
}

int ctx_outputs(blsv_ctx* c, size_t n, bool with_cls, PassOut& out) {
  HIPCHK(c, c->bitmap.ensure((n + 63) / 64 * 8 + 8));
  HIPCHK(c, c->first_bad.ensure(8));
  HIPCHK(c, hipMemsetAsync(c->first_bad.p, 0xff, 8, c->stream));
  if (with_cls) HIPCHK(c, c->misc.ensure(n + 64));
  out = {c->bitmap.as<uint64_t>(), c->first_bad.as<unsigned long long>(), with_cls ? c->misc.as<uint8_t>() : nullptr, 0};
  return BLSV_OK;
}

using LatFn = std::function<void(uint8_t* cls)>;

static int verify_host(blsv_ctx* c, size_t n, const SigSrc& sig, const PkSel& pk, const HashFn& hash, const LatFn& lat,
                       bool randomized, uint64_t first_round, const uint64_t* rounds, uint8_t* ok_bitmap,
                       uint64_t* first_bad, uint8_t* reject_class) {
  auto put_first_bad = [&](uint64_t fb) {
    if (first_bad) *first_bad = fb == UINT64_MAX ? fb : rounds ? rounds[fb] : first_round + fb;
  };
  int rc = ensure_workspace(c, n);
  if (rc) return rc;
  if (use_lat(c, n)) {
    {
      StageTimer tm(c, ST_LAT, n, c->stream);
      lat(c->cls.as<uint8_t>());
    }
    HIPCHK(c, hipGetLastError());
    std::vector<uint8_t> own;
    uint8_t* cls = reject_class;
    if (!cls) {
      own.resize(n);
      cls = own.data();
    }
    HIPCHK(c, download_sync(c, {{cls, c->cls.p, n}}));
    put_first_bad(fold_classes(cls, n, ok_bitmap));
    return BLSV_OK;
  }
  Tail tail;
  tail.randomized = randomized;
  if (randomized && (rc = rlc_draw_seed(c, tail.seed))) return rc;
  PassOut out;
  rc = ctx_outputs(c, n, reject_class != nullptr, out);
  if (rc) return rc;
  rc = run_passes(c, n, sig, pk, hash, tail, out, c->stream);
  if (rc) return rc;
  const size_t words = (n + 63) / 64;
  std::vector<uint64_t> w(words + 1, 0);
  uint64_t fb = UINT64_MAX;
  HIPCHK(c, download_sync(c, {{w.data(), c->bitmap.p, words * 8},
                              {&fb, c->first_bad.p, 8},
                              {reject_class, c->misc.p, reject_class ? n : 0}}));
  if (ok_bitmap) bitmap_words_to_bytes(w.data(), n, ok_bitmap);
  put_first_bad(fb);
  return BLSV_OK;
}

int decode_g1(blsv_ctx* c, const uint8_t* pk48, size_t cnt, DBuf& tab, DBuf& inf, std::vector<uint8_t>& cls) {
  HIPCHK(c, tab.ensure(cnt * blsk::G1_WORDS * 4));
  HIPCHK(c, inf.ensure(cnt));
  HIPCHK(c, c->g1_cls.ensure(cnt));
  HIPCHK(c, c->misc.ensure(cnt * 48));
  HIPCHK(c, hipMemcpyAsync(c->misc.p, pk48, cnt * 48, hipMemcpyHostToDevice, c->stream));
  blsk::launch_decompress_g1(c->misc.as<uint8_t>(), cnt, tab.as<uint32_t>(), inf.as<uint8_t>(),
                             c->g1_cls.as<uint8_t>(), c->stream);
  HIPCHK(c, hipGetLastError());
  cls.assign(cnt, 0);
  HIPCHK(c, hipMemcpyAsync(cls.data(), c->g1_cls.p, cnt, hipMemcpyDeviceToHost, c->stream));
  HIPCHK(c, hipStreamSynchronize(c->stream));
  return BLSV_OK;
}

int upload_messages(blsv_ctx* c, const uint8_t* msgs, const uint32_t* msg_lens, size_t n) {
  std::vector<uint64_t> off(n + 1, 0);
  for (size_t i = 0; i < n; i++) off[i + 1] = off[i] + msg_lens[i];
  if (off[n] && !msgs) return fail(c, BLSV_EINVAL, "messages: %llu message bytes but no buffer",
                                   (unsigned long long)off[n]);
  HIPCHK(c, c->in_msgs.ensure(off[n] + 1));
  HIPCHK(c, c->in_off.ensure((n + 1) * 8));
  HIPCHK(c, c->in_len.ensure(n * 4 + 4));
  const size_t staged_max = kIoCap / 4;
  HIPCHK(c, h2d(c, c->in_msgs.p, msgs, off[n]));
  HIPCHK(c, h2d(c, c->in_off.p, off.data(), (n + 1) * 8));
  HIPCHK(c, h2d(c, c->in_len.p, msg_lens, n * 4));
  if ((n + 1) * 8 > staged_max) HIPCHK(c, hipStreamSynchronize(c->stream));
  return BLSV_OK;
}

int svc_verify_mixed(blsv_ctx* c, size_t n, const uint8_t* msgs, const uint64_t* off, const uint32_t* lens,
                     const uint8_t* sigs96, const uint32_t* idx, const uint32_t* d_tab, const uint8_t* d_tab_inf,
                     uint8_t* cls_out) {
  if (!n) return BLSV_OK;
  if (n > kMaxChunk) return fail(c, BLSV_EINVAL, "service batch larger than %zu", kMaxChunk);
  (void)hipSetDevice(c->device);
  int rc = ensure_workspace(c, std::min(n, c->chunk));
  if (rc) return rc;
  const size_t mbytes = off[n];
  const SvcLayout l = svc_layout(n, mbytes);
  HIPCHK(c, c->pin.ensure(std::max(l.total, n + 8)));
  uint8_t* h = c->pin.as<uint8_t>();
  memcpy(h, off, (n + 1) * 8);
  memcpy(h + l.o_len, lens, n * 4);
  memcpy(h + l.o_idx, idx, n * 4);
  memcpy(h + l.o_sig, sigs96, n * 96);
  if (mbytes) memcpy(h + l.o_msg, msgs, mbytes);
  HIPCHK(c, c->arena.ensure(l.total));
  HIPCHK(c, c->misc.ensure(n + 64));
  HIPCHK(c, hipMemcpyAsync(c->arena.p, h, l.total, hipMemcpyHostToDevice, c->stream));
  uint8_t* d = c->arena.as<uint8_t>();
  const uint64_t* d_off = reinterpret_cast<const uint64_t*>(d);
  const uint32_t* d_len = reinterpret_cast<const uint32_t*>(d + l.o_len);
  const uint8_t* d_msg = d + l.o_msg;
  const SigSrc sig{d + l.o_sig, 96, 0};
  const PkSel pk{d_tab, d_tab_inf, reinterpret_cast<const uint32_t*>(d + l.o_idx)};
  if (use_lat(c, n)) {
    blsk::launch_lat_messages(d_msg, d_off, d_len, sig.d, 96, 0, n, pk.tab, pk.inf, pk.idx, c->misc.as<uint8_t>(),
                              nullptr, nullptr, c->stream);
  } else {
    PassOut out;
    rc = ctx_outputs(c, n, true, out);
    if (rc) return rc;
    rc = run_passes(
        c, n, sig, pk,
        [&](size_t base, size_t cnt, hipStream_t st) { hash_messages(c, d_msg, d_off, d_len, base, cnt, st); }, Tail(),
        out, c->stream);
    if (rc) return rc;
  }
  HIPCHK(c, hipGetLastError());
  HIPCHK(c, hipMemcpyAsync(h, c->misc.p, n, hipMemcpyDeviceToHost, c->stream));
  HIPCHK(c, hipStreamSynchronize(c->stream));
  memcpy(cls_out, h, n);
  return BLSV_OK;
}

int stage_chain(blsv_ctx* c, uint64_t first_round, const uint8_t* prevs, size_t prev0_len, bool prev_rows,
                const uint8_t* sigs96, size_t n, blsk::ChainedSrc& src) {
  HIPCHK(c, c->in_sigs.ensure(n * 96 + 96));
  HIPCHK(c, c->seeds.ensure(prev_rows ? n * 96 + 96 : 96));
  if (n) {
    HIPCHK(c, h2d(c, c->in_sigs.p, sigs96, n * 96));
    HIPCHK(c, h2d(c, c->seeds.p, prevs, prev_rows ? n * 96 : prev0_len));
  }
  src = {c->in_sigs.as<uint8_t>(), c->seeds.as<uint8_t>(), first_round, prev_rows ? 1 : std::max<uint64_t>(n, 1),
         (uint32_t)prev0_len};
  return BLSV_OK;
}

static int chained_host(blsv_ctx* c, const char* name, bool prev_rows, bool randomized, uint64_t first_round,
                        const uint8_t* prevs, size_t prev0_len, const uint8_t* sigs96, size_t n, uint8_t* ok_bitmap,
                        uint64_t* first_bad, uint8_t* reject_class) {
  if (!c->has_group) return fail(c, BLSV_ENOGROUP, "%s: no group key set", name);
  if (n && (!sigs96 || !prevs || (prev0_len != 32 && prev0_len != 96)))
    return fail(c, BLSV_EINVAL, "%s: %s must be 32 or 96 bytes", name, prev_rows ? "row 0's prev" : "prev0");
  if (n > SIZE_MAX / 96 - 1) return fail(c, BLSV_EINVAL, "%s: %zu rounds overflow the byte count", name, n);
  (void)hipSetDevice(c->device);
  blsk::ChainedSrc src;
  const int rc = stage_chain(c, first_round, prevs, prev0_len, prev_rows, sigs96, n, src);
  if (rc) return rc;
  const PkSel pk = group_pk(c);
  return verify_host(
      c, n, {src.sigs, 96, 0}, pk, [&](size_t base, size_t cnt, hipStream_t st) { hash_chained(c, src, base, cnt, st); },
      [&](uint8_t* cls) { blsk::launch_lat_chained(src, 0, n, pk.tab, pk.inf, cls, c->stream); }, randomized,
      first_round, nullptr, ok_bitmap, first_bad, reject_class);
}

static int unchained_host(blsv_ctx* c, const char* name, bool randomized, const uint64_t* rounds, uint64_t first_round,
                          const uint8_t* sigs96, size_t n, uint8_t* ok_bitmap, uint64_t* first_bad,
                          uint8_t* reject_class) {
  if (!c->has_group) return fail(c, BLSV_ENOGROUP, "%s: no group key set", name);
  if (n && !sigs96) return fail(c, BLSV_EINVAL, "%s: null signatures", name);
  (void)hipSetDevice(c->device);
  HIPCHK(c, c->in_sigs.ensure(n * 96 + 96));
  if (n) HIPCHK(c, h2d(c, c->in_sigs.p, sigs96, n * 96));
  const uint64_t* d_rounds = nullptr;
  if (rounds && n) {
    HIPCHK(c, c->in_rounds.ensure(n * 8));
    HIPCHK(c, h2d(c, c->in_rounds.p, rounds, n * 8));
    d_rounds = c->in_rounds.as<uint64_t>();
  }
  const PkSel pk = group_pk(c);
  const SigSrc sig{c->in_sigs.as<uint8_t>(), 96, 0};
  return verify_host(
      c, n, sig, pk,
      [&](size_t base, size_t cnt, hipStream_t st) {
        const Staging w = staging(c);
        blsk::launch_hash_unchained(d_rounds, first_round, base, cnt, w.H, w.h_inf, w.HQ, st);
      },
      [&](uint8_t* cls) { blsk::launch_lat_unchained(d_rounds, first_round, sig.d, 0, n, pk.tab, pk.inf, cls, c->stream); },
      randomized, first_round, rounds, ok_bitmap, first_bad, reject_class);
}

static int run_lat(blsv_ctx* c, size_t n, const LatFn& lat, const PassOut& out, hipStream_t st) {
  {
    StageTimer tm(c, ST_LAT, n, st);
    lat(c->cls.as<uint8_t>());
  }
  blsk::launch_finish(c->cls.as<uint8_t>(), 0, n, out.bitmap, out.first_bad, out.label0, st);
  if (out.cls) HIPCHK(c, hipMemcpyAsync(out.cls, c->cls.p, n, hipMemcpyDeviceToDevice, st));
  HIPCHK(c, hipGetLastError());
  return BLSV_OK;
}

static int chained_dev(blsv_ctx* c, const char* name, bool randomized, uint64_t first_round, uint64_t seg_len,
                       uint64_t seg_phase, const uint8_t* d_seeds96, size_t seed0_len, const uint8_t* d_sigs96, size_t n,
                       uint64_t* d_bitmap, uint64_t* d_first_bad, uint8_t* d_reject_class, void* stream) {
  if (!c->has_group) return fail(c, BLSV_ENOGROUP, "%s: no group key set", name);
  if (n && (!d_seeds96 || !d_sigs96 || !d_bitmap || !d_first_bad || (seed0_len != 32 && seed0_len != 96)))
    return fail(c, BLSV_EINVAL, "%s: bad arguments", name);
  if (seg_phase && (!seg_len || seg_phase >= seg_len))
    return fail(c, BLSV_EINVAL, "%s: seg_phase must be < seg_len", name);
  (void)hipSetDevice(c->device);
  hipStream_t st = stream ? (hipStream_t)stream : c->stream;
  Tail tail;
  tail.randomized = randomized;
  int rc = randomized ? rlc_draw_seed(c, tail.seed) : BLSV_OK;
  if (rc) return rc;
  HIPCHK(c, hipMemsetAsync(d_first_bad, 0xff, 8, st));
  rc = ensure_workspace(c, n);
  if (rc) return rc;
  const blsk::ChainedSrc src{d_sigs96,           d_seeds96, first_round, seg_len ? seg_len : std::max<uint64_t>(n, 1),
                             (uint32_t)seed0_len, seg_phase};
  const PkSel pk = group_pk(c);
  const PassOut out{d_bitmap, (unsigned long long*)d_first_bad, d_reject_class, first_round};
  if (use_lat(c, n))
    return run_lat(c, n, [&](uint8_t* cls) { blsk::launch_lat_chained(src, 0, n, pk.tab, pk.inf, cls, st); }, out, st);
  return run_passes(
      c, n, {d_sigs96, 96, 0}, pk, [&](size_t base, size_t cnt, hipStream_t s) { hash_chained(c, src, base, cnt, s); },
      tail, out, st);
}

extern "C" {

int blsv_verify_chained(blsv_ctx* c, uint64_t first_round, const uint8_t* prev0, size_t prev0_len,
                        const uint8_t* sigs96, size_t n, uint8_t* ok_bitmap, uint64_t* first_bad,
                        uint8_t* reject_class) {
  if (!c) return BLSV_EINVAL;
  return chained_host(c, "verify_chained", false, false, first_round, prev0, prev0_len, sigs96, n, ok_bitmap, first_bad,
                      reject_class);
}

int blsv_verify_prevs(blsv_ctx* c, uint64_t first_round, const uint8_t* prevs96, size_t prev0_len,
                      const uint8_t* sigs96, size_t n, uint8_t* ok_bitmap, uint64_t* first_bad,
                      uint8_t* reject_class) {
  if (!c) return BLSV_EINVAL;
  return chained_host(c, "verify_prevs", true, false, first_round, prevs96, prev0_len, sigs96, n, ok_bitmap, first_bad,
                      reject_class);
}

int blsv_verify_chained_rlc(blsv_ctx* c, uint64_t first_round, const uint8_t* prev0, size_t prev0_len,
                            const uint8_t* sigs96, size_t n, uint8_t* ok_bitmap, uint64_t* first_bad,
                            uint8_t* reject_class) {
  if (!c) return BLSV_EINVAL;
  const bool rlc = use_rlc(c, n);
  return chained_host(c, rlc ? "verify_chained_rlc" : "verify_chained", false, rlc, first_round, prev0, prev0_len,
                      sigs96, n, ok_bitmap, first_bad, reject_class);
}

int blsv_verify_unchained(blsv_ctx* c, const uint64_t* rounds, uint64_t first_round, const uint8_t* sigs96, size_t n,
                          uint8_t* ok_bitmap, uint64_t* first_bad, uint8_t* reject_class) {
  if (!c) return BLSV_EINVAL;
  return unchained_host(c, "verify_unchained", false, rounds, first_round, sigs96, n, ok_bitmap, first_bad,
                        reject_class);
}

int blsv_verify_unchained_rlc(blsv_ctx* c, const uint64_t* rounds, uint64_t first_round, const uint8_t* sigs96,
                              size_t n, uint8_t* ok_bitmap, uint64_t* first_bad, uint8_t* reject_class) {
  if (!c) return BLSV_EINVAL;
  const bool rlc = use_rlc(c, n);
  return unchained_host(c, rlc ? "verify_unchained_rlc" : "verify_unchained", rlc, rounds, first_round, sigs96, n,
                        ok_bitmap, first_bad, reject_class);
}

int blsv_verify_chained_dev(blsv_ctx* c, uint64_t first_round, uint64_t seg_len, uint64_t seg_phase,
                            const uint8_t* d_seeds96, size_t seed0_len, const uint8_t* d_sigs96, size_t n,
                            uint64_t* d_bitmap, uint64_t* d_first_bad, uint8_t* d_reject_class, void* stream) {
  if (!c) return BLSV_EINVAL;
  return chained_dev(c, "verify_chained_dev", false, first_round, seg_len, seg_phase, d_seeds96, seed0_len, d_sigs96, n,
                     d_bitmap, d_first_bad, d_reject_class, stream);
}

int blsv_verify_chained_rlc_dev(blsv_ctx* c, uint64_t first_round, uint64_t seg_len, uint64_t seg_phase,
                                const uint8_t* d_seeds96, size_t seed0_len, const uint8_t* d_sigs96, size_t n,
                                uint64_t* d_bitmap, uint64_t* d_first_bad, uint8_t* d_reject_class, void* stream) {
  if (!c) return BLSV_EINVAL;
  const bool rlc = use_rlc(c, n);
  return chained_dev(c, rlc ? "verify_chained_rlc_dev" : "verify_chained_dev", rlc, first_round, seg_len, seg_phase,
                     d_seeds96, seed0_len, d_sigs96, n, d_bitmap, d_first_bad, d_reject_class, stream);
}

int blsv_verify_chained_multi(blsv_ctx* const* ctxs, size_t n_ctx, const size_t* shard_counts, uint64_t first_round,
                              const uint8_t* prev0, size_t prev0_len, const uint8_t* sigs96, size_t n,
                              uint8_t* ok_bitmap, uint64_t* first_bad, uint8_t* reject_class) {
  if (!ctxs || n_ctx == 0) return BLSV_EINVAL;
  for (size_t k = 0; k < n_ctx; k++) {
    if (!ctxs[k]) return BLSV_EINVAL;
    for (size_t j = 0; j < k; j++)
      if (ctxs[j] == ctxs[k]) return fail(ctxs[k], BLSV_EINVAL, "verify_chained_multi: context %zu repeated", k);
  }
  blsv_ctx* c0 = ctxs[0];
  for (size_t k = 0; k < n_ctx; k++) {
    if (!ctxs[k]->has_group) return fail(ctxs[k], BLSV_ENOGROUP, "verify_chained_multi: context %zu has no group", k);
    if (ctxs[k]->group_bytes != c0->group_bytes)
      return fail(ctxs[k], BLSV_EINVAL, "verify_chained_multi: context %zu holds another group", k);
  }
  if (n && (!sigs96 || !prev0 || (prev0_len != 32 && prev0_len != 96)))
    return fail(c0, BLSV_EINVAL, "verify_chained_multi: prev0 must be 32 or 96 bytes");
  std::vector<size_t> cnt(n_ctx), start(n_ctx);
  size_t sum = 0;
  for (size_t k = 0; k < n_ctx; k++) {
    cnt[k] = shard_counts ? shard_counts[k] : n / n_ctx + (k < n % n_ctx ? 1 : 0);
    start[k] = sum;
    sum += cnt[k];
  }
  if (sum != n) return fail(c0, BLSV_EINVAL, "verify_chained_multi: shard counts sum to %zu, not %zu", sum, n);
  std::vector<std::vector<uint8_t>> bms(n_ctx);
  std::vector<uint64_t> fbs(n_ctx, UINT64_MAX);
  std::vector<int> rcs(n_ctx, BLSV_OK);
  auto shard = [&](size_t k) {
    if (!cnt[k]) return;
    bms[k].assign((cnt[k] + 7) / 8, 0);
    const bool head = start[k] == 0;
    const uint8_t* halo = head ? prev0 : sigs96 + (start[k] - 1) * 96;
    rcs[k] = blsv_verify_chained(ctxs[k], first_round + start[k], halo, head ? prev0_len : 96, sigs96 + start[k] * 96,
                                 cnt[k], bms[k].data(), &fbs[k], reject_class ? reject_class + start[k] : nullptr);
  };
  std::vector<std::thread> th;
  for (size_t k = 1; k < n_ctx; k++)
    if (cnt[k]) th.emplace_back(shard, k);
  shard(0);
  for (auto& t : th) t.join();
  for (size_t k = 0; k < n_ctx; k++)
    if (rcs[k]) return rcs[k];
  uint64_t fb = UINT64_MAX;
  for (size_t k = 0; k < n_ctx; k++) fb = std::min(fb, fbs[k]);
  if (first_bad) *first_bad = fb;
  if (ok_bitmap && n) {
    memset(ok_bitmap, 0, (n + 7) / 8);
    for (size_t k = 0; k < n_ctx; k++)
      if (cnt[k]) or_bits_at(ok_bitmap, bms[k].data(), cnt[k], start[k]);
  }
  return BLSV_OK;
}

int blsv_verify_messages(blsv_ctx* c, const uint8_t* pk48, const uint8_t* msgs, const uint32_t* msg_lens, size_t n,
                         const uint8_t* sigs96, uint8_t* ok_bitmap, uint64_t* first_bad, uint8_t* reject_class) {
  if (!c) return BLSV_EINVAL;
  if (n && (!msg_lens || !sigs96)) return fail(c, BLSV_EINVAL, "verify_messages: null arguments");
  (void)hipSetDevice(c->device);
  PkSel pk;
  if (pk48) {
    if (!c->pk_cache_valid || memcmp(c->pk_cache, pk48, 48) != 0) {
      std::vector<uint8_t> cls;
      int rc = decode_g1(c, pk48, 1, c->pk_tab, c->pk_inf, cls);
      if (rc) return rc;
      if (cls[0]) return fail(c, BLSV_EINVAL, "verify_messages: public key rejected (class %d)", (int)cls[0]);
      memcpy(c->pk_cache, pk48, 48);
      c->pk_cache_valid = true;
    }
    pk = {c->pk_tab.as<uint32_t>(), c->pk_inf.as<uint8_t>(), nullptr};
  } else {
    if (!c->has_group) return fail(c, BLSV_ENOGROUP, "verify_messages: no group key set");
    pk = group_pk(c);
  }
  if (n > kMaxChunk) return fail(c, BLSV_EINVAL, "verify_messages: batch larger than %zu", kMaxChunk);
  int rc = upload_messages(c, msgs, msg_lens, n);
  if (rc) return rc;
  HIPCHK(c, c->in_sigs.ensure(n * 96 + 96));
  if (n) HIPCHK(c, h2d(c, c->in_sigs.p, sigs96, n * 96));
  const SigSrc sig{c->in_sigs.as<uint8_t>(), 96, 0};
  return verify_host(
      c, n, sig, pk, [&](size_t base, size_t cnt, hipStream_t st) { hash_uploaded(c, base, cnt, st); },
      [&](uint8_t* cls) { lat_uploaded(c, sig, n, pk, cls, nullptr, nullptr, c->stream); }, false, 0, nullptr, ok_bitmap,
      first_bad, reject_class);
}

int blsv_generate_chained_dev(blsv_ctx* c, const uint8_t* sk32, uint64_t first_round, uint64_t seg_len,
                              const uint8_t* d_seeds96, size_t seed0_len, uint8_t* d_sigs96, size_t n, void* stream) {
  if (!c) return BLSV_EINVAL;
  if (!sk32 || (n && (!d_seeds96 || !d_sigs96)) || (seed0_len != 32 && seed0_len != 96))
    return fail(c, BLSV_EINVAL, "generate_chained_dev: bad arguments");
  (void)hipSetDevice(c->device);
  hipStream_t st = stream ? (hipStream_t)stream : c->stream;
  uint32_t sk[8];
  scalar_mod_r(sk32, sk);
  HIPCHK(c, c->sk.ensure(32));
  HIPCHK(c, hipMemcpyAsync(c->sk.p, sk, 32, hipMemcpyHostToDevice, st));
  blsk::ChainedSrc src{d_sigs96, d_seeds96, first_round, seg_len ? seg_len : std::max<uint64_t>(n, 1),
                       (uint32_t)seed0_len};
  blsk::launch_gen_chained(c->sk.as<uint32_t>(), src, n, d_sigs96, st);
  HIPCHK(c, hipGetLastError());
  HIPCHK(c, hipStreamSynchronize(st));
  return BLSV_OK;
}

size_t blsv_set_rlc_group(blsv_ctx* c, size_t g) {
  if (!c) return 0;
  const size_t prev = c->rlc.group;
  size_t v = kRlcGroupMin;
  while (v * 2 <= g && v < kRlcGroupMax) v *= 2;
  c->rlc.group = v;
  return prev;
}

int blsv_rlc_stats(blsv_ctx* c, uint64_t* groups, uint64_t* groups_failed, uint64_t* items_exact) {
  if (!c) return BLSV_EINVAL;
  if (groups) *groups = c->rlc.groups;
  if (groups_failed) *groups_failed = c->rlc.groups_failed;
  if (items_exact) *items_exact = c->rlc.items_exact;
  return BLSV_OK;
}

}
```

drand_amd/engine.py:

```python
from __future__ import annotations

import ctypes
from dataclasses import dataclass

from . import _lib
from ._lib import u8p, u32p, u64p


class EngineError(RuntimeError):
    def __init__(self, code, msg):
        super().__init__(f"blsverify error {code}: {msg}")
        self.code = code


@dataclass
class BatchResult:
    ok: list
    first_bad: int | None
    reject_class: list

    @property
    def all_ok(self):
        return self.first_bad is None

    def bitmap(self):
        out = bytearray((len(self.ok) + 7) // 8)
        for i, v in enumerate(self.ok):
            if v:
                out[i // 8] |= 1 << (i % 8)
        return bytes(out)


class SignatureRejected(EngineError):

    def __init__(self, code, msg, sig_class):
        super().__init__(code, msg)
        self.sig_class = sig_class


@dataclass
class TlockResult:
    ok: list
    reject_class: list
    gt: list


def _bits(bitmap, n):
    import numpy as np
    if n == 0:
        return []
    return np.unpackbits(np.frombuffer(bytes(bitmap), np.uint8), bitorder="little")[:n].astype(bool).tolist()


class Engine:

    def __init__(self, device: int = 0, init_torch: bool = True):
        if init_torch:
            try:
                import torch
            except ImportError:
                torch = None
            if torch is not None:
                torch.cuda.set_device(int(device))
                torch.zeros(1, device=torch.device("cuda", int(device)))
        self.lib = _lib.load()
        h = ctypes.c_void_p()
        rc = self.lib.blsv_create(int(device), ctypes.byref(h))
        if rc != 0:
            raise EngineError(rc, f"blsv_create(device={device}) failed")
        self._h = h
        self._ops = None
        self.device = device

    def close(self):
        if getattr(self, "_h", None) is not None and self._h.value:
            self.lib.blsv_destroy(self._h)
            self._h = None

    def __del__(self):
        try:
            self.close()
        except Exception:
            pass

    def __enter__(self):
        return self

    def __exit__(self, *exc):
        self.close()

    def _check(self, rc):
        if rc != 0:
            raise EngineError(rc, self.lib.blsv_last_error(self._h).decode())
        return rc

    @property
    def handle(self):
        return self._h

    def synchronize(self):
        self._check(self.lib.blsv_synchronize(self._h))

    def set_group(self, commits, n=None):
        commits = [bytes(c) for c in commits]
        if any(len(c) != 48 for c in commits):
            raise ValueError("commitments must be 48 bytes")
        t = len(commits)
        self._check(self.lib.blsv_set_group(self._h, _lib.buf(b"".join(commits)), t, n if n is not None else t))

    def set_public_key(self, pk48):
        self.set_group([pk48], 1)

    def verify_chained(self, first_round, prev0, sigs):
        n = len(sigs)
        sigb = b"".join(bytes(s) for s in sigs)
        if any(len(s) != 96 for s in sigs):
            raise ValueError("chained signatures must be 96 bytes (reject wrong lengths host-side)")
        bm = _lib.out_buf((n + 7) // 8)
        fb = ctypes.c_uint64()
        cls = _lib.out_buf(n)
        self._check(self.lib.blsv_verify_chained(self._h, first_round, _lib.buf(prev0), len(prev0), _lib.buf(sigb), n,
                                                 bm, ctypes.byref(fb), cls))
        return BatchResult(_bits(bm, n), None if fb.value == 2 ** 64 - 1 else fb.value, list(cls)[:n])

    def verify_chained_packed(self, first_round, prev0, sigs96, n):
        mv = memoryview(sigs96).cast("B")
        if len(mv) != 96 * n:
            raise ValueError("packed signatures must be n*96 bytes")
        bm = _lib.out_buf((n + 7) // 8)
        fb = ctypes.c_uint64()
        cls = _lib.out_buf(n)
        src = (ctypes.c_uint8 * max(len(mv), 1)).from_buffer_copy(mv) if len(mv) else None
        self._check(self.lib.blsv_verify_chained(self._h, first_round, _lib.buf(prev0), len(prev0), src, n, bm,
                                                 ctypes.byref(fb), cls))
        return BatchResult(_bits(bm, n), None if fb.value == 2 ** 64 - 1 else fb.value, list(cls)[:n])

    def verify_prevs(self, first_round, prev0_len, prevs96, sigs96, n):
        import numpy as np
        p = np.ascontiguousarray(np.frombuffer(memoryview(prevs96).cast("B"), np.uint8))
        q = np.ascontiguousarray(np.frombuffer(memoryview(sigs96).cast("B"), np.uint8))
        if len(p) != 96 * n or len(q) != 96 * n:
            raise ValueError("prevs and sigs must be n*96 bytes")
        bm = np.zeros(max((n + 7) // 8, 1), np.uint8)
        cls = np.zeros(max(n, 1), np.uint8)
        fb = ctypes.c_uint64()
        u8 = ctypes.POINTER(ctypes.c_uint8)
        ptr = lambda a: a.ctypes.data_as(u8) if a.size else None
        self._check(self.lib.blsv_verify_prevs(self._h, first_round, ptr(p), prev0_len, ptr(q), n, ptr(bm),
                                               ctypes.byref(fb), ptr(cls)))
        ok = np.unpackbits(bm, bitorder="little")[:n].astype(bool)
        return BatchResult(ok, None if fb.value == 2 ** 64 - 1 else fb.value, cls[:n])

    def verify_unchained(self, sigs, first_round=None, rounds=None):
        n = len(sigs)
        if any(len(s) != 96 for s in sigs):
            raise ValueError("signatures must be 96 bytes (reject wrong lengths host-side)")
        sigb = b"".join(bytes(s) for s in sigs)
        rr = None
        if rounds is not None:
            rr = (ctypes.c_uint64 * max(n, 1))(*rounds)
        bm = _lib.out_buf((n + 7) // 8)
        fb = ctypes.c_uint64()
        cls = _lib.out_buf(n)
        self._check(self.lib.blsv_verify_unchained(self._h, rr, first_round or 0, _lib.buf(sigb), n, bm,
                                                   ctypes.byref(fb), cls))
        return BatchResult(_bits(bm, n), None if fb.value == 2 ** 64 - 1 else fb.value, list(cls)[:n])

    def verify_messages(self, msgs, sigs, pk48=None):
        n = len(msgs)
        assert len(sigs) == n
        if any(len(s) != 96 for s in sigs):
            raise ValueError("signatures must be 96 bytes (reject wrong lengths host-side)")
        lens = (ctypes.c_uint32 * max(n, 1))(*[len(m) for m in msgs])
        bm = _lib.out_buf((n + 7) // 8)
        fb = ctypes.c_uint64()
        cls = _lib.out_buf(n)
        self._check(self.lib.blsv_verify_messages(self._h, _lib.buf(pk48) if pk48 is not None else None,
                                                  _lib.buf(b"".join(bytes(m) for m in msgs)), lens, n,
                                                  _lib.buf(b"".join(bytes(s) for s in sigs)), bm, ctypes.byref(fb),
                                                  cls))
        return BatchResult(_bits(bm, n), None if fb.value == 2 ** 64 - 1 else fb.value, list(cls)[:n])

    def verify_partials(self, msg, partials):
        k = len(partials)
        plen = len(partials[0]) if k else 98
        if any(len(p) != plen for p in partials):
            raise ValueError("partials of one call must share a length")
        ok = _lib.out_buf(k)
        cls = _lib.out_buf(k)
        self._check(self.lib.blsv_verify_partials(self._h, _lib.buf(msg), len(msg),
                                                  _lib.buf(b"".join(bytes(p) for p in partials)), plen, k, ok, cls))
        return [bool(x) for x in list(ok)[:k]], list(cls)[:k]

    def verify_partials_multi(self, msgs, partials):
        k = len(partials)
        assert len(msgs) == k
        plen = len(partials[0]) if k else 98
        if any(len(p) != plen for p in partials):
            raise ValueError("partials of one call must share a length")
        lens = (ctypes.c_uint32 * max(k, 1))(*[len(m) for m in msgs])
        ok = _lib.out_buf(k)
        cls = _lib.out_buf(k)
        self._check(self.lib.blsv_verify_partials_multi(self._h, _lib.buf(b"".join(bytes(m) for m in msgs)), lens,
                                                        _lib.buf(b"".join(bytes(p) for p in partials)), plen, k, ok,
                                                        cls))
        return [bool(x) for x in list(ok)[:k]], list(cls)[:k]

    def recover(self, msg, partials, t, n):
        k = len(partials)
        plen = len(partials[0]) if k else 98
        out = _lib.out_buf(96)
        self._check(self.lib.blsv_recover(self._h, _lib.buf(msg), len(msg),
                                          _lib.buf(b"".join(bytes(p) for p in partials)), plen, k, t, n, out))
        return bytes(out)

    def aggregate(self, msg, partials, t, n):
        k = len(partials)
        plen = len(partials[0]) if k else 98
        if any(len(p) != plen for p in partials):
            raise ValueError("partials of one call must share a length")
        ok = _lib.out_buf(k)
        cls = _lib.out_buf(k)
        out = _lib.out_buf(96)
        gok = _lib.out_buf(1)
        self._check(self.lib.blsv_aggregate(self._h, _lib.buf(msg), len(msg),
                                            _lib.buf(b"".join(bytes(p) for p in partials)), plen, k, t, n, ok, cls,
                                            out, gok))
        return [bool(x) for x in list(ok)[:k]], list(cls)[:k], bytes(out), bool(gok[0])

    def aggregate_round(self, msg1, partials1, msg2, partials2, t, n):
        bad_share = b"\xff\xff" + bytes(96)
        partials1 = [p if len(p) == 98 else bad_share for p in (bytes(p) for p in partials1)]
        partials2 = [p if len(p) == 98 else bad_share for p in (bytes(p) for p in partials2)]
        k1, k2 = len(partials1), len(partials2)
        plen = 98
        ok1, ok2 = _lib.out_buf(k1), _lib.out_buf(k2)
        s1, s2 = _lib.out_buf(96), _lib.out_buf(96)
        st = ctypes.c_int32()
        v2 = _lib.out_buf(1)
        self._check(self.lib.blsv_aggregate_round(
            self._h, _lib.buf(msg1), len(msg1), _lib.buf(b"".join(partials1)), k1,
            _lib.buf(msg2), len(msg2), _lib.buf(b"".join(partials2)), k2, plen, t, n, ok1, ok2,
            s1, s2, ctypes.byref(st), v2))
        status = st.value
        sig1 = bytes(s1) if status in (_lib.AGG_OK, _lib.AGG_OK_V2, _lib.AGG_V1_INVALID,
                                       _lib.AGG_V2_RECOVER_FAIL) else None
        sig2 = bytes(s2) if status == _lib.AGG_OK_V2 else None
        r1 = [bool(x) for x in list(ok1)[:k1]]
        r2 = [bool(x) for x in list(ok2)[:k2]]
        return status, r1, r2, sig1, sig2, bool(v2[0])

    def sign(self, sk32, msgs, index=-1):
        n = len(msgs)
        lens = (ctypes.c_uint32 * max(n, 1))(*[len(m) for m in msgs])
        stride = 98 if index >= 0 else 96
        out = _lib.out_buf(n * stride)
        self._check(self.lib.blsv_sign(self._h, _lib.buf(sk32), index, _lib.buf(b"".join(bytes(m) for m in msgs)),
                                       lens, n, out))
        ob = bytes(out)
        return [ob[i * stride:(i + 1) * stride] for i in range(n)]

    def verify_chained_dev(self, first_round, seg_len, d_seeds, seed0_len, d_sigs, n, d_bitmap, d_first_bad,
                           d_cls=None, stream=None, seg_phase=0):
        self._check(self.lib.blsv_verify_chained_dev(self._h, first_round, seg_len, seg_phase, d_seeds, seed0_len,
                                                     d_sigs, n, d_bitmap, d_first_bad, d_cls, stream))

    def generate_chained_dev(self, sk32, first_round, seg_len, d_seeds, seed0_len, d_sigs, n, stream=None):
        self._check(self.lib.blsv_generate_chained_dev(self._h, _lib.buf(sk32), first_round, seg_len, d_seeds,
                                                       seed0_len, d_sigs, n, stream))

    def verify_chained_rlc(self, first_round, prev0, sigs):
        n = len(sigs)
        if any(len(s) != 96 for s in sigs):
            raise ValueError("chained signatures must be 96 bytes (reject wrong lengths host-side)")
        sigb = b"".join(bytes(s) for s in sigs)
        bm = _lib.out_buf((n + 7) // 8)
        fb = ctypes.c_uint64()
        cls = _lib.out_buf(n)
        self._check(self.lib.blsv_verify_chained_rlc(self._h, first_round, _lib.buf(prev0), len(prev0), _lib.buf(sigb),
                                                     n, bm, ctypes.byref(fb), cls))
        return BatchResult(_bits(bm, n), None if fb.value == 2 ** 64 - 1 else fb.value, list(cls)[:n])

    def verify_unchained_rlc(self, sigs, first_round=None, rounds=None):
        n = len(sigs)
        if any(len(s) != 96 for s in sigs):
            raise ValueError("signatures must be 96 bytes (reject wrong lengths host-side)")
        sigb = b"".join(bytes(s) for s in sigs)
        rr = None
        if rounds is not None:
            rr = (ctypes.c_uint64 * max(n, 1))(*rounds)
        bm = _lib.out_buf((n + 7) // 8)
        fb = ctypes.c_uint64()
        cls = _lib.out_buf(n)
        self._check(self.lib.blsv_verify_unchained_rlc(self._h, rr, first_round or 0, _lib.buf(sigb), n, bm,
                                                       ctypes.byref(fb), cls))
        return BatchResult(_bits(bm, n), None if fb.value == 2 ** 64 - 1 else fb.value, list(cls)[:n])

    def verify_chained_rlc_dev(self, first_round, seg_len, d_seeds, seed0_len, d_sigs, n, d_bitmap, d_first_bad,
                               d_cls=None, stream=None, seg_phase=0):
        self._check(self.lib.blsv_verify_chained_rlc_dev(self._h, first_round, seg_len, seg_phase, d_seeds, seed0_len,
                                                         d_sigs, n, d_bitmap, d_first_bad, d_cls, stream))

    def set_rlc_group(self, g):
        return self.lib.blsv_set_rlc_group(self._h, int(g))

    def rlc_stats(self):
        a, b, c = ctypes.c_uint64(), ctypes.c_uint64(), ctypes.c_uint64()
        self._check(self.lib.blsv_rlc_stats(self._h, ctypes.byref(a), ctypes.byref(b), ctypes.byref(c)))
        return a.value, b.value, c.value

    def test_rlc_seed(self, seed32):
        if seed32 is not None and len(seed32) != 32:
            raise ValueError("the seed is 32 bytes")
        self._check(self.lib.blsv_test_rlc_seed(self._h, _lib.buf(seed32) if seed32 is not None else None))

    def test_rlc_sums(self, first_round, prev0, sigs):
        n = len(sigs)
        sigb = b"".join(bytes(s) for s in sigs)
        cap = -(-n // 8) + n // 16384 + 1
        a, b = _lib.out_buf(cap * 96), _lib.out_buf(cap * 96)
        ng = self.lib.blsv_test_rlc_sums(self._h, first_round, _lib.buf(prev0), len(prev0), _lib.buf(sigb), n, a, b)
        if ng < 0:
            raise EngineError(ng, self.lib.blsv_last_error(self._h).decode())
        ab, bb = bytes(a), bytes(b)
        return ([ab[96 * k:96 * k + 96] for k in range(ng)], [bb[96 * k:96 * k + 96] for k in range(ng)])

    def tlock_open(self, sig, us):
        sig = bytes(sig)
        us = [bytes(u) for u in us]
        if len(sig) != 96:
            raise ValueError("the round signature is 96 bytes")
        if any(len(u) != 48 for u in us):
            raise ValueError("U values must be 48 bytes (reject wrong lengths host-side)")
        n = len(us)
        out = _lib.out_buf(n * 576)
        ok = _lib.out_buf(n)
        cls = _lib.out_buf(n)
        sc = ctypes.c_uint8()
        rc = self.lib.blsv_tlock_open(self._h, _lib.buf(sig), _lib.buf(b"".join(us)), n, out, ok, cls,
                                      ctypes.cast(ctypes.byref(sc), u8p))
        if rc == _lib.BLSV_EINVAL and sc.value:
            raise SignatureRejected(rc, self.lib.blsv_last_error(self._h).decode(), sc.value)
        self._check(rc)
        ob = bytes(out)
        oks = [bool(x) for x in list(ok)[:n]]
        return TlockResult(oks, list(cls)[:n], [ob[576 * i:576 * i + 576] if oks[i] else None for i in range(n)])

    def tlock_open_dev(self, sig, d_us, n, d_out, d_cls=None, stream=None):
        sig = bytes(sig)
        if len(sig) != 96:
            raise ValueError("the round signature is 96 bytes")
        self._check(self.lib.blsv_tlock_open_dev(self._h, _lib.buf(sig), d_us, n, d_out, d_cls, stream))

    def tlock_stats(self):
        a, b = ctypes.c_uint64(), ctypes.c_uint64()
        self._check(self.lib.blsv_tlock_stats(self._h, ctypes.byref(a), ctypes.byref(b)))
        return a.value, b.value

    STAGES = ("hash", "decompress", "miller", "final_exp", "finish", "lat", "rlc", "tlock")

    def profile(self, on=True):
        self._check(self.lib.blsv_profile_enable(self._h, 1 if on else 0))

    def profile_read(self):
        n = len(self.STAGES)
        ms = (ctypes.c_double * n)()
        la = (ctypes.c_uint64 * n)()
        it = (ctypes.c_uint64 * n)()
        rc = self.lib.blsv_profile_read(self._h, ms, la, it, n)
        if rc < 0:
            raise EngineError(rc, self.lib.blsv_last_error(self._h).decode())
        return {s: (ms[k], la[k], it[k]) for k, s in enumerate(self.STAGES)}

    LAT_MARKS = ("start", "hash", "sig_decoded", "sig_miller", "phase_a", "key_miller", "miller_product",
                 "final_exp", "pow1_start", "pow1_end", "xmd_done", "sswu_done", "iso_add_done", "cofactor_done",
                 "sig_sqrt_done", "sig_subgroup_done")

    def lat_trace_enable(self, on=True):
        self._check(self.lib.blsv_lat_trace_enable(self._h, 1 if on else 0))

    def lat_trace(self, clear=True):
        n = len(self.LAT_MARKS)
        t = (ctypes.c_uint64 * n)()
        rate = ctypes.c_double()
        got = self.lib.blsv_lat_trace(self._h, t, n, ctypes.byref(rate), 1 if clear else 0)
        if got < 0:
            raise EngineError(got, self.lib.blsv_last_error(self._h).decode())
        t0 = t[0]
        return {k: (t[i] - t0) / rate.value for i, k in enumerate(self.LAT_MARKS[:got]) if t[i] and t0}

    def set_lat_max(self, n):
        return self.lib.blsv_set_lat_max(self._h, int(n))

    def set_chunk(self, items):
        return self.lib.blsv_set_chunk(self._h, int(items))

    def workspace_bytes(self):
        return self.lib.blsv_workspace_bytes(self._h)

    def test_fp_mul(self, a_limbs, b_limbs):
        n = len(a_limbs) // 12
        A = (ctypes.c_uint32 * max(len(a_limbs), 1))(*a_limbs)
        B = (ctypes.c_uint32 * max(len(b_limbs), 1))(*b_limbs)
        O = (ctypes.c_uint32 * max(n * 12, 1))()
        self._check(self.lib.blsv_test_fp_mul(self._h, A, B, n, O))
        return list(O)[:n * 12]

    def test_ops(self):
        ops, k = {}, 0
        name, a, b, c = ctypes.c_char_p(), ctypes.c_int(), ctypes.c_int(), ctypes.c_int()
        while self.lib.blsv_test_op_info(k, ctypes.byref(name), ctypes.byref(a), ctypes.byref(b), ctypes.byref(c)) == 0:
            ops[name.value.decode()] = (a.value, b.value, c.value)
            k += 1
        return ops

    def test_op(self, name, operands):
        if self._ops is None:
            self._ops = self.test_ops()
        nin, nout, _ = self._ops[name]
        if len(operands) % nin:
            raise ValueError(f"{name} takes {nin} Fp elements per item")
        n = len(operands) // nin
        raw = b"".join(int(v).to_bytes(48, "little") for v in operands)
        A = (ctypes.c_uint32 * max(len(raw) // 4, 1)).from_buffer_copy(raw if raw else bytes(4))
        O = (ctypes.c_uint32 * max(n * nout * 12, 1))()
        self._check(self.lib.blsv_test_op(self._h, name.encode(), A, n, O))
        ob = bytes(O)
        return [int.from_bytes(ob[48 * k:48 * k + 48], "little") for k in range(n * nout)]

    def test_pairing(self, p_words, q_words):
        n = len(p_words) // 24
        Pp = (ctypes.c_uint32 * max(len(p_words), 1))(*p_words)
        Q = (ctypes.c_uint32 * max(len(q_words), 1))(*q_words)
        O = (ctypes.c_uint32 * max(n * 144, 1))()
        self._check(self.lib.blsv_test_pairing(self._h, Pp, Q, n, O))
        return list(O)[:n * 144]

    def test_final_exp(self, f_words):
        n = len(f_words) // 144
        Fw = (ctypes.c_uint32 * max(len(f_words), 1))(*f_words)
        A = (ctypes.c_uint32 * max(n * 144, 1))()
        B = (ctypes.c_uint32 * max(n * 144, 1))()
        self._check(self.lib.blsv_test_final_exp(self._h, Fw, n, A, B))
        return list(A)[:n * 144], list(B)[:n * 144]

    def test_hash_to_g2(self, msgs):
        n = len(msgs)
        lens = (ctypes.c_uint32 * max(n, 1))(*[len(m) for m in msgs])
        O = (ctypes.c_uint32 * max(n * 48, 1))()
        inf = _lib.out_buf(n)
        self._check(self.lib.blsv_test_hash_to_g2(self._h, _lib.buf(b"".join(bytes(m) for m in msgs)), lens, n, O,
                                                  inf))
        return list(O)[:n * 48], list(inf)[:n]

    def spec_stats(self):
        h, m = ctypes.c_uint64(), ctypes.c_uint64()
        self._check(self.lib.blsv_test_spec_stats(self._h, ctypes.byref(h), ctypes.byref(m)))
        return h.value, m.value

    def test_generic_chains(self, on=True):
        self._check(self.lib.blsv_test_generic_chains(self._h, 1 if on else 0))


def verify_chained_multi(engines, first_round, prev0, sigs, counts=None):
    if not engines:
        raise ValueError("verify_chained_multi needs at least one engine")
    lib = engines[0].lib
    n = len(sigs)
    if any(len(s) != 96 for s in sigs):
        raise ValueError("chained signatures must be 96 bytes (reject wrong lengths host-side)")
    sigb = b"".join(bytes(s) for s in sigs)
    hs = (ctypes.c_void_p * len(engines))(*[e._h.value for e in engines])
    cs = None if counts is None else (ctypes.c_size_t * len(engines))(*counts)
    bm = _lib.out_buf((n + 7) // 8)
    fb = ctypes.c_uint64()
    cls = _lib.out_buf(n)
    rc = lib.blsv_verify_chained_multi(hs, len(engines), cs, first_round, _lib.buf(prev0), len(prev0), _lib.buf(sigb),
                                       n, bm, ctypes.byref(fb), cls)
    if rc != 0:
        msgs = "; ".join(lib.blsv_last_error(e._h).decode(errors="replace") for e in engines)
        raise EngineError(rc, f"blsv_verify_chained_multi failed: {msgs}")
    return BatchResult(_bits(bm, n), None if fb.value == 2 ** 64 - 1 else fb.value, list(cls)[:n])


class Service:

    def __init__(self, device: int = 0, gap_us: int = 0, max_wait_us: int = 0, init_torch: bool = True):
        if init_torch:
            try:
                import torch
            except ImportError:
                torch = None
            if torch is not None:
                torch.cuda.set_device(int(device))
                torch.zeros(1, device=torch.device("cuda", int(device)))
        self.lib = _lib.load()
        h = ctypes.c_void_p()
        rc = self.lib.blsv_service_create(int(device), int(gap_us), int(max_wait_us), ctypes.byref(h))
        if rc != 0:
            raise EngineError(rc, f"blsv_service_create(device={device}) failed")
        self._h = h

    def close(self):
        if getattr(self, "_h", None) is not None and self._h.value:
            self.lib.blsv_service_destroy(self._h)
            self._h = None

    def __enter__(self):
        return self

    def __exit__(self, *exc):
        self.close()

    def verify_partial(self, commits, n, msg, partial):
        cb = b"".join(bytes(c) for c in commits)
        ok, cls = ctypes.c_uint8(), ctypes.c_uint8()
        p = bytes(partial)
        rc = self.lib.blsv_service_verify_partial(self._h, _lib.buf(cb), len(commits), int(n), _lib.buf(msg), len(msg),
                                                  _lib.buf(p), len(p), ctypes.byref(ok), ctypes.byref(cls))
        if rc != 0:
            raise EngineError(rc, "blsv_service_verify_partial failed")
        return bool(ok.value), cls.value

    def prepare_partial(self, commits, n, msg, partial):
        cb = _lib.buf(b"".join(bytes(c) for c in commits))
        mb, pb = _lib.buf(msg), _lib.buf(bytes(partial))
        t, ml, pl = len(commits), len(msg), len(partial)
        ok, cls = ctypes.c_uint8(), ctypes.c_uint8()
        f, h, pok, pcls = self.lib.blsv_service_verify_partial, self._h, ctypes.byref(ok), ctypes.byref(cls)

        def call():
            rc = f(h, cb, t, n, mb, ml, pb, pl, pok, pcls)
            if rc != 0:
                raise EngineError(rc, "blsv_service_verify_partial failed")
            return bool(ok.value), cls.value

        return call

    def verify_recovered(self, pk48, msg, sig96):
        ok, cls = ctypes.c_uint8(), ctypes.c_uint8()
        rc = self.lib.blsv_service_verify_recovered(self._h, _lib.buf(pk48), _lib.buf(msg), len(msg), _lib.buf(sig96),
                                                    ctypes.byref(ok), ctypes.byref(cls))
        if rc != 0:
            raise EngineError(rc, "blsv_service_verify_recovered failed")
        return bool(ok.value), cls.value

    def test_limits(self, chunk=0, lat_max=(1 << 64) - 1, arena_entries=0):
        n = ctypes.c_uint64()
        rc = self.lib.blsv_test_service_limits(self._h, int(chunk), int(lat_max), int(arena_entries), ctypes.byref(n))
        if rc != 0:
            raise EngineError(rc, "blsv_test_service_limits failed")
        return n.value

    def stats(self):
        a, b, c = ctypes.c_uint64(), ctypes.c_uint64(), ctypes.c_uint64()
        self.lib.blsv_service_stats(self._h, ctypes.byref(a), ctypes.byref(b), ctypes.byref(c))
        return a.value, b.value, c.value


def limbs_of(v, n=12):
    return [(v >> (32 * i)) & 0xFFFFFFFF for i in range(n)]


def int_of(limbs):
    return sum(int(x) << (32 * i) for i, x in enumerate(limbs))
```

include/blsverify_testing.h:

```cpp
#ifndef DRAND_AMD_BLSVERIFY_TESTING_H
#define DRAND_AMD_BLSVERIFY_TESTING_H

#include "blsverify.h"

#ifdef __cplusplus
extern "C" {
#endif

int blsv_test_fp_mul(blsv_ctx* ctx, const uint32_t* a, const uint32_t* b, size_t n, uint32_t* out);

int blsv_test_pairing(blsv_ctx* ctx, const uint32_t* p, const uint32_t* q, size_t n, uint32_t* out_f);

int blsv_test_final_exp(blsv_ctx* ctx, const uint32_t* f, size_t n, uint32_t* out_pipeline, uint32_t* out_ref);

int blsv_test_op(blsv_ctx* ctx, const char* name, const uint32_t* in, size_t n, uint32_t* out);
int blsv_test_op_info(int index, const char** name, int* in_fp, int* out_fp, int* lanes);

int blsv_test_hash_to_g2(blsv_ctx* ctx, const uint8_t* msgs, const uint32_t* msg_lens, size_t n, uint32_t* out,
                         uint8_t* inf);

int blsv_test_generic_chains(blsv_ctx* ctx, int on);

int blsv_test_spec_stats(blsv_ctx* ctx, uint64_t* hits, uint64_t* misses);

int blsv_test_service_limits(blsv_service* svc, size_t chunk, size_t lat_max, size_t arena_entries,
                             uint64_t* sub_launches);

int blsv_profile_enable(blsv_ctx* ctx, int on);
int blsv_lat_trace(blsv_ctx* ctx, uint64_t* ticks, int n, double* ticks_per_us, int clear);
int blsv_lat_trace_enable(blsv_ctx* ctx, int on);
int blsv_profile_read(blsv_ctx* ctx, double* ms, uint64_t* launches, uint64_t* items, int nstages);
int blsv_test_lagrange(const uint32_t* idx, size_t t, uint32_t* out);

int blsv_test_rlc_seed(blsv_ctx* ctx, const uint8_t* seed32);
int blsv_test_rlc_sums(blsv_ctx* ctx, uint64_t first_round, const uint8_t* prev0, size_t prev0_len,
                       const uint8_t* sigs96, size_t n, uint8_t* out_a96, uint8_t* out_b96);

#ifdef __cplusplus
}
#endif

#endif
```

Measured before the change: 2.412 million beacons/s.

## Split pairing tail remainder onto side stream to overlap with main batch

The pairing check now splits its items into a main part that is a multiple of a device-derived quantum (64*4*CUs) and a remainder. The remainder runs Miller-f (single-lane) and final exponentiation on a side stream, concurrently with the main part's final exponentiation, and the two are joined with events. The aim is to fill idle CUs during the partial last wave. In exchange, final-exp park buffers are offset inside HQ (workspace resized), profiling records gain paired events, and cross-stream synchronisation adds overhead. The split applies only when the count is at most the line-sub size and not a multiple of the quantum.

```diff
diff --git a/drand_amd/_lib.py b/drand_amd/_lib.py
--- a/drand_amd/_lib.py
+++ b/drand_amd/_lib.py
@@ -80,6 +80,7 @@
     "blsv_test_pairing": (ctypes.c_int, [vp, u32p, u32p, sz, u32p]),
     "blsv_test_hash_to_g2": (ctypes.c_int, [vp, u8p, u32p, sz, u32p, u8p]),
     "blsv_test_final_exp": (ctypes.c_int, [vp, u32p, sz, u32p, u32p]),
+    "blsv_test_tail_split": (ctypes.c_int, [vp, sz]),
     "blsv_set_lat_max": (sz, [vp, sz]),
     "blsv_set_chunk": (sz, [vp, sz]),
     "blsv_workspace_bytes": (sz, [vp]),
diff --git a/drand_amd/csrc/blsverify.cpp b/drand_amd/csrc/blsverify.cpp
--- a/drand_amd/csrc/blsverify.cpp
+++ b/drand_amd/csrc/blsverify.cpp
@@ -15,7 +15,7 @@
       if (e == hipSuccess) e = d.ensure(bytes);
     };
     need(c->H, want * blsk::H_WORDS * 4);
-    need(c->HQ, want * blsk::HQ_WORDS * 4);
+    need(c->HQ, kHqWords(want) * 4);
     need(c->S, want * blsk::S_WORDS * 4);
     need(c->F, want * blsk::F_WORDS * 4);
     need(c->FW, 3 * want * blsk::F_WORDS * 4);
@@ -113,6 +113,9 @@
     if (e == hipSuccess) e = hipEventCreateWithFlags(&ev, hipEventDisableTiming);
   if (e == hipSuccess) e = hipEventCreateWithFlags(&c->fork_ev, hipEventDisableTiming);
   if (e == hipSuccess) e = hipEventCreateWithFlags(&c->join_ev, hipEventDisableTiming);
+  int cus = 0;
+  if (e == hipSuccess) e = hipDeviceGetAttribute(&cus, hipDeviceAttributeMultiprocessorCount, device);
+  c->tail_q_dev = c->tail_q = size_t(64) * 4 * (size_t)std::max(cus, 0);
   if (e != hipSuccess) {
     fprintf(stderr, "blsv_create: %s\n", hipGetErrorString(e));
     blsv_destroy(c);
@@ -135,10 +138,9 @@
   if (c->fork_ev) (void)hipEventDestroy(c->fork_ev);
   if (c->join_ev) (void)hipEventDestroy(c->join_ev);
   (void)hipDeviceSynchronize();
-  for (auto& r : c->recs) {
-    (void)hipEventDestroy(r.a);
-    (void)hipEventDestroy(r.b);
-  }
+  for (auto& r : c->recs)
+    for (hipEvent_t e : {r.a, r.b, r.a2, r.b2})
+      if (e) (void)hipEventDestroy(e);
   for (auto e : c->event_pool) (void)hipEventDestroy(e);
   delete c;
 }
@@ -169,13 +171,19 @@
     HIPCHK(c, hipEventSynchronize(r.b));
     float t = 0;
     HIPCHK(c, hipEventElapsedTime(&t, r.a, r.b));
+    if (r.a2 && r.b2) {
+      float t2 = 0;
+      HIPCHK(c, hipEventSynchronize(r.b2));
+      HIPCHK(c, hipEventElapsedTime(&t2, r.a2, r.b2));
+      t += t2;
+    }
     if (r.stage < nstages) {
       if (ms) ms[r.stage] += t;
       if (launches) launches[r.stage] += 1;
       if (items) items[r.stage] += r.items;
     }
-    c->event_pool.push_back(r.a);
-    c->event_pool.push_back(r.b);
+    for (hipEvent_t e : {r.a, r.b, r.a2, r.b2})
+      if (e) c->event_pool.push_back(e);
   }
   c->recs.clear();
   return ST_N;
diff --git a/drand_amd/csrc/engine_ctx.h b/drand_amd/csrc/engine_ctx.h
--- a/drand_amd/csrc/engine_ctx.h
+++ b/drand_amd/csrc/engine_ctx.h
@@ -19,8 +19,11 @@
 constexpr size_t kMinChunk = size_t(1) << 14;
 constexpr size_t kLineSub = kMaxChunk;
 constexpr size_t kPkTable = 4096;
+constexpr size_t kFexpParkWords(size_t items) { return blsk::FEXP_PARK_WORDS(items) + 48 * 64; }
+constexpr size_t kHqWords(size_t items) { return std::max(items * blsk::HQ_WORDS, kFexpParkWords(items)); }
 constexpr size_t kStagingBytesPerItem =
-    4 * (blsk::H_WORDS + blsk::HQ_WORDS + blsk::S_WORDS + 4 * blsk::F_WORDS + blsk::MILLER_LINE_WORDS) + 3;
+    4 * (blsk::H_WORDS + blsk::HQ_WORDS + 3 + blsk::S_WORDS + 4 * blsk::F_WORDS + blsk::MILLER_LINE_WORDS) + 3;
+static_assert(kHqWords(kMaxChunk) <= (blsk::HQ_WORDS + 3) * kMaxChunk, "kStagingBytesPerItem: HQ with the park");
 static_assert(576ull * kMaxChunk < 0x7fffffffull, "SoA object resource exceeds its 31-bit num_records");
 static_assert((133ull * kMaxChunk) * 4 < 0xffffffffull, "SoA VGPR byte offset exceeds 32 bits");
 static_assert(48ull * 4 * kMaxChunk < 0x7fffffffull, "3-lane park slot resource exceeds 31 bits");
@@ -98,6 +101,7 @@
   int stage;
   size_t items;
   hipEvent_t a, b;
+  hipEvent_t a2 = nullptr, b2 = nullptr;
 };
 
 constexpr size_t kRlcGroupDefault = 64;
@@ -160,6 +164,7 @@
   size_t chunk = chunk_env();
   size_t lat_max = std::min(lat_max_env(), chunk);
   uint64_t oom_halvings = 0;
+  size_t tail_q_dev = 0, tail_q = 0;
   std::vector<ProfRec> recs;
   std::vector<hipEvent_t> event_pool;
   hipStream_t stream = nullptr;
diff --git a/drand_amd/csrc/host_internal.h b/drand_amd/csrc/host_internal.h
--- a/drand_amd/csrc/host_internal.h
+++ b/drand_amd/csrc/host_internal.h
@@ -73,9 +73,13 @@
   blsk::launch_lat_messages(c->in_msgs.as<uint8_t>(), c->in_off.as<uint64_t>(), c->in_len.as<uint32_t>(), sig.d,
                             sig.stride, sig.offset, cnt, pk.tab, pk.inf, pk.idx, cls, S, s_inf, st);
 }
+inline void final_exp(blsv_ctx* c, size_t cnt, size_t base, size_t m, uint8_t* cls, hipStream_t st,
+                      uint32_t* out = nullptr) {
+  const Staging w = staging(c);
+  blsk::launch_final_exp(w.F, w.FW, cnt, base, m, cls, st, w.HQ + (base ? blsk::FEXP_PARK_WORDS(base) : 0), out);
+}
 inline void final_exp(blsv_ctx* c, size_t cnt, uint8_t* cls, hipStream_t st, uint32_t* out = nullptr) {
-  const Staging w = staging(c);
-  blsk::launch_final_exp(w.F, w.FW, cnt, cls, st, w.LN, out);
+  final_exp(c, cnt, 0, cnt, cls, st, out);
 }
 
 inline bool use_lat(const blsv_ctx* c, size_t n) { return n > 0 && n <= std::min(c->lat_max, c->cap); }
diff --git a/drand_amd/csrc/hostlogic.h b/drand_amd/csrc/hostlogic.h
--- a/drand_amd/csrc/hostlogic.h
+++ b/drand_amd/csrc/hostlogic.h
@@ -221,6 +221,11 @@
   return nf * G - (fail[nf - 1] == ng - 1 ? ng * G - cnt : 0);
 }
 
+inline size_t tail_split_main(size_t cnt, size_t q) {
+  if (q == 0 || cnt <= q || cnt % q == 0) return cnt;
+  return cnt - cnt % q;
+}
+
 struct SvcLayout {
   size_t o_len, o_idx, o_sig, o_msg, total;
 };
diff --git a/drand_amd/csrc/k_fexp.hip b/drand_amd/csrc/k_fexp.hip
--- a/drand_amd/csrc/k_fexp.hip
+++ b/drand_amd/csrc/k_fexp.hip
@@ -2,10 +2,10 @@
 
 namespace blsk {
 
-BLS_KERNEL(BLS_WPE_FEXP) k_fexp_easy(const uint32_t* F, size_t cnt, const uint8_t* cls, uint32_t* G) {
+BLS_KERNEL(BLS_WPE_FEXP) k_fexp_easy(const uint32_t* F, size_t n, size_t m, const uint8_t* cls, uint32_t* G) {
   size_t i = (size_t)blockIdx.x * TPB + threadIdx.x;
-  if (i >= cnt || cls[i] != REJ_OK) return;
-  st_fp12(G, cnt, i, fexp_easy(ld_fp12(F, cnt, i)));
+  if (i >= m || cls[i] != REJ_OK) return;
+  st_fp12(G, n, i, fexp_easy(ld_fp12(F, n, i)));
 }
 
 #ifndef BLS_WPE_FEXP_TRI
@@ -32,21 +32,21 @@
 }
 
 template <int MODE>
-BLS_KERNEL(BLS_WPE_FEXP_TRI) k_fexp_tri(const uint32_t* X, const uint32_t* C, const uint32_t* G, size_t cnt,
+BLS_KERNEL(BLS_WPE_FEXP_TRI) k_fexp_tri(const uint32_t* X, const uint32_t* C, const uint32_t* G, size_t n, size_t m,
                                         uint8_t* cls, uint32_t* OUT, uint32_t* park) {
   const tri_lane t = tri_lane_id();
 #if BLS_CSQR_LIN
   kp_lds_init<11>();
 #endif
   const size_t ir = (size_t)blockIdx.x * TRI_GROUPS + t.group;
-  const bool in_range = t.group < TRI_GROUPS && ir < cnt;
-  const size_t i0 = in_range ? ir : cnt - 1;
+  const bool in_range = t.group < TRI_GROUPS && ir < m;
+  const size_t i0 = in_range ? ir : m - 1;
   const bool live = in_range && cls[i0] == REJ_OK;
   const TriPark pk = {park, (size_t)gridDim.x * TPB, (size_t)blockIdx.x * TPB + t.lane};
   auto at = [&](const uint32_t* B) {
     size_t j = i0;
     asm volatile("" : "+v"(j));
-    return tri_load(B, cnt, j, t.role);
+    return tri_load(B, n, j, t.role);
   };
   fp4 r = tri_conj(t, tri_pow_x_abs(t, [&]() { return at(X); }, pk));
   if (MODE == 0 || MODE == 1) r = tri_mul_lp(t, r, tri_conj(t, at(X)), pk.p, pk.n, pk.i);
@@ -58,7 +58,7 @@
     r = tri_mul_lp(t, r, at(G), pk.p, pk.n, pk.i);
   }
   if (MODE < 4 || OUT) {
-    if (live) tri_store(OUT, cnt, i0, t.role, r);
+    if (live) tri_store(OUT, n, i0, t.role, r);
   }
   if (MODE == 4) {
     const bool one = tri_is_one(t, r);
@@ -66,20 +66,23 @@
   }
 }
 
-void launch_final_exp(uint32_t* F, uint32_t* W, size_t cnt, uint8_t* cls, hipStream_t st, uint32_t* park,
-                      uint32_t* out) {
-  if (!cnt) return;
-  uint32_t* G = W;
-  uint32_t* B = W + cnt * F_WORDS;
-  uint32_t* C = W + 2 * cnt * F_WORDS;
-  const dim3 grid(grid_for(cnt)), blk(TPB);
-  hipLaunchKernelGGL(k_fexp_easy, grid, blk, 0, st, F, cnt, cls, G);
-  const dim3 tgrid((unsigned)((cnt + TRI_GROUPS - 1) / TRI_GROUPS));
-  hipLaunchKernelGGL(k_fexp_tri<0>, tgrid, blk, 0, st, G, nullptr, nullptr, cnt, cls, F, park);
-  hipLaunchKernelGGL(k_fexp_tri<1>, tgrid, blk, 0, st, F, nullptr, nullptr, cnt, cls, B, park);
-  hipLaunchKernelGGL(k_fexp_tri<2>, tgrid, blk, 0, st, B, nullptr, nullptr, cnt, cls, C, park);
-  hipLaunchKernelGGL(k_fexp_tri<3>, tgrid, blk, 0, st, C, nullptr, nullptr, cnt, cls, F, park);
-  hipLaunchKernelGGL(k_fexp_tri<4>, tgrid, blk, 0, st, F, C, G, cnt, cls, out, park);
+void launch_final_exp(uint32_t* F, uint32_t* W, size_t n, size_t base, size_t m, uint8_t* cls, hipStream_t st,
+                      uint32_t* park, uint32_t* out) {
+  if (!m) return;
+  F += base;
+  cls += base;
+  if (out) out += base;
+  uint32_t* G = W + base;
+  uint32_t* B = G + n * F_WORDS;
+  uint32_t* C = G + 2 * n * F_WORDS;
+  const dim3 grid(grid_for(m)), blk(TPB);
+  hipLaunchKernelGGL(k_fexp_easy, grid, blk, 0, st, F, n, m, cls, G);
+  const dim3 tgrid((unsigned)((m + TRI_GROUPS - 1) / TRI_GROUPS));
+  hipLaunchKernelGGL(k_fexp_tri<0>, tgrid, blk, 0, st, G, nullptr, nullptr, n, m, cls, F, park);
+  hipLaunchKernelGGL(k_fexp_tri<1>, tgrid, blk, 0, st, F, nullptr, nullptr, n, m, cls, B, park);
+  hipLaunchKernelGGL(k_fexp_tri<2>, tgrid, blk, 0, st, B, nullptr, nullptr, n, m, cls, C, park);
+  hipLaunchKernelGGL(k_fexp_tri<3>, tgrid, blk, 0, st, C, nullptr, nullptr, n, m, cls, F, park);
+  hipLaunchKernelGGL(k_fexp_tri<4>, tgrid, blk, 0, st, F, C, G, n, m, cls, out, park);
 }
 
 }
diff --git a/drand_amd/csrc/k_miller.hip b/drand_amd/csrc/k_miller.hip
--- a/drand_amd/csrc/k_miller.hip
+++ b/drand_amd/csrc/k_miller.hip
@@ -298,25 +298,39 @@
   return true;
 }
 
+void launch_miller_lines(const uint32_t* pk_tab, const uint8_t* pk_inf, const uint32_t* pk_idx, const uint32_t* H,
+                         const uint8_t* h_inf, const uint32_t* S, const uint8_t* s_inf, uint8_t* cls, size_t cnt,
+                         size_t base, size_t m, uint32_t* LN, size_t sub, bool check_subgroup, hipStream_t st) {
+  if (!m) return;
+  if (check_subgroup)
+    hipLaunchKernelGGL(k_miller_lines<true>, dim3(2 * grid_for(m)), dim3(TPB), 0, st, pk_tab, pk_inf, pk_idx, H, h_inf,
+                       S, s_inf, cls, cnt, base, m, sub, LN);
+  else
+    hipLaunchKernelGGL(k_miller_lines<false>, dim3(2 * grid_for(m)), dim3(TPB), 0, st, pk_tab, pk_inf, pk_idx, H,
+                       h_inf, S, s_inf, (const uint8_t*)cls, cnt, base, m, sub, LN);
+}
+
+void launch_miller_f(const uint32_t* LN, size_t sub, const uint8_t* cls, size_t cnt, size_t base, size_t m,
+                     uint32_t* F, uint32_t* park, bool single_lane, hipStream_t st) {
+  if (!m) return;
+  LN += base % sub;
+  if (m <= kMillerTriMax && !single_lane) {
+    hipLaunchKernelGGL(k_miller_f_tri, dim3((unsigned)((m + TRI_GROUPS - 1) / TRI_GROUPS)), dim3(TPB), 0, st, LN, cls,
+                       cnt, base, m, sub, F, park);
+  } else {
+    hipLaunchKernelGGL(k_miller_f, dim3(grid_for(m)), dim3(TPB), 0, st, LN, cls, cnt, base, m, sub, F);
+  }
+}
+
 void launch_miller(const uint32_t* pk_tab, const uint8_t* pk_inf, const uint32_t* pk_idx, const uint32_t* H,
                    const uint8_t* h_inf, const uint32_t* S, const uint8_t* s_inf, uint8_t* cls, size_t cnt,
                    uint32_t* F, uint32_t* LN, size_t sub, uint32_t* park, bool check_subgroup, hipStream_t st) {
   if (!cnt) return;
   for (size_t b = 0; b < cnt; b += sub) {
     const size_t m = cnt - b < sub ? cnt - b : sub;
-    if (check_subgroup)
-      hipLaunchKernelGGL(k_miller_lines<true>, dim3(2 * grid_for(m)), dim3(TPB), 0, st, pk_tab, pk_inf, pk_idx, H,
-                         h_inf, S, s_inf, cls, cnt, b, m, sub, LN);
-    else
-      hipLaunchKernelGGL(k_miller_lines<false>, dim3(2 * grid_for(m)), dim3(TPB), 0, st, pk_tab, pk_inf, pk_idx, H,
-                         h_inf, S, s_inf, (const uint8_t*)cls, cnt, b, m, sub, LN);
-    if (m <= kMillerTriMax) {
-      hipLaunchKernelGGL(k_miller_f_tri, dim3((unsigned)((m + TRI_GROUPS - 1) / TRI_GROUPS)), dim3(TPB), 0, st, LN,
-                         cls, cnt, b, m, sub, F, park);
-    } else {
-      hipLaunchKernelGGL(k_miller_f, dim3(grid_for(m)), dim3(TPB), 0, st, LN, cls, cnt, b, m, sub, F);
-    }
-  }
-}
-
-}
+    launch_miller_lines(pk_tab, pk_inf, pk_idx, H, h_inf, S, s_inf, cls, cnt, b, m, LN, sub, check_subgroup, st);
+    launch_miller_f(LN, sub, cls, cnt, b, m, F, park, false, st);
+  }
+}
+
+}
diff --git a/drand_amd/csrc/kernels.h b/drand_amd/csrc/kernels.h
--- a/drand_amd/csrc/kernels.h
+++ b/drand_amd/csrc/kernels.h
@@ -32,10 +32,15 @@
 void launch_miller(const uint32_t* pk_tab, const uint8_t* pk_inf, const uint32_t* pk_idx, const uint32_t* H,
                    const uint8_t* h_inf, const uint32_t* S, const uint8_t* s_inf, uint8_t* cls, size_t cnt,
                    uint32_t* F, uint32_t* LN, size_t sub, uint32_t* park, bool check_subgroup, hipStream_t st);
+void launch_miller_lines(const uint32_t* pk_tab, const uint8_t* pk_inf, const uint32_t* pk_idx, const uint32_t* H,
+                         const uint8_t* h_inf, const uint32_t* S, const uint8_t* s_inf, uint8_t* cls, size_t cnt,
+                         size_t base, size_t m, uint32_t* LN, size_t sub, bool check_subgroup, hipStream_t st);
+void launch_miller_f(const uint32_t* LN, size_t sub, const uint8_t* cls, size_t cnt, size_t base, size_t m,
+                     uint32_t* F, uint32_t* park, bool single_lane, hipStream_t st);
 constexpr size_t TRI_PARK_WORDS(size_t items) { return 48 * 64 * ((items + 20) / 21); }
 constexpr size_t FEXP_PARK_WORDS(size_t items) { return TRI_PARK_WORDS(items); }
-void launch_final_exp(uint32_t* F, uint32_t* W, size_t cnt, uint8_t* cls, hipStream_t st, uint32_t* park,
-                      uint32_t* out = nullptr);
+void launch_final_exp(uint32_t* F, uint32_t* W, size_t n, size_t base, size_t m, uint8_t* cls, hipStream_t st,
+                      uint32_t* park, uint32_t* out = nullptr);
 void launch_finish(const uint8_t* cls, size_t base, size_t cnt, uint64_t* bitmap, unsigned long long* first_bad,
                    uint64_t label0, hipStream_t st);
 
diff --git a/drand_amd/csrc/testhooks.cpp b/drand_amd/csrc/testhooks.cpp
--- a/drand_amd/csrc/testhooks.cpp
+++ b/drand_amd/csrc/testhooks.cpp
@@ -77,6 +77,12 @@
   return BLSV_OK;
 }
 
+int blsv_test_tail_split(blsv_ctx* c, size_t q) {
+  if (!c) return BLSV_EINVAL;
+  c->tail_q = q == SIZE_MAX ? c->tail_q_dev : q;
+  return BLSV_OK;
+}
+
 int blsv_test_generic_chains(blsv_ctx* c, int on) {
   if (!c) return BLSV_EINVAL;
   blsk::g_generic_chains_all = on != 0;
@@ -158,7 +164,9 @@
   HIPCHK(c, hipMemsetAsync(w.cls, 0, n, c->stream));
   blsk::launch_test_pack_fp12(din.as<uint32_t>(), n, w.F, c->stream);
   blsk::launch_test_final_exp_ref(w.F, n, dref.as<uint32_t>(), c->stream);
-  final_exp(c, n, w.cls, c->stream, dout.as<uint32_t>());
+  const size_t mn = tail_split_main(n, c->tail_q);
+  final_exp(c, n, 0, mn, w.cls, c->stream, dout.as<uint32_t>());
+  final_exp(c, n, mn, n - mn, w.cls, c->stream, dout.as<uint32_t>());
   blsk::launch_test_unpack_fp12(dout.as<uint32_t>(), n, din.as<uint32_t>(), c->stream);
   HIPCHK(c, hipMemcpyAsync(out_pipeline, din.p, n * 576, hipMemcpyDeviceToHost, c->stream));
   blsk::launch_test_unpack_fp12(dref.as<uint32_t>(), n, dout.as<uint32_t>(), c->stream);
diff --git a/drand_amd/csrc/tlock.cpp b/drand_amd/csrc/tlock.cpp
--- a/drand_amd/csrc/tlock.cpp
+++ b/drand_amd/csrc/tlock.cpp
@@ -49,7 +49,7 @@
   }
   {
     StageTimer tm(c, ST_FEXP, cnt, st);
-    final_exp(c, cnt, w.cls, st, w.HQ);
+    blsk::launch_final_exp(w.F, w.FW, cnt, 0, cnt, w.cls, st, w.LN, w.HQ);
   }
   blsk::launch_tlock_encode(w.HQ, ucls, cnt, d_out, st);
   if (d_cls_out) HIPCHK(c, hipMemcpyAsync(d_cls_out, ucls, cnt, hipMemcpyDeviceToDevice, st));
diff --git a/drand_amd/csrc/verify.cpp b/drand_amd/csrc/verify.cpp
--- a/drand_amd/csrc/verify.cpp
+++ b/drand_amd/csrc/verify.cpp
@@ -46,16 +46,76 @@
   return BLSV_OK;
 }
 
-static void pairing_check(blsv_ctx* c, const PkSel& pk, const uint32_t* H, const uint8_t* h_inf, const uint32_t* S,
-                          const uint8_t* s_inf, uint8_t* cls, size_t cnt, bool check_subgroup, hipStream_t st) {
+struct SplitDrain {
+  blsv_ctx* c;
+  bool armed = false;
+  ~SplitDrain() {
+    if (armed) (void)hipStreamSynchronize(c->side);
+  }
+};
+
+static int pairing_check(blsv_ctx* c, const PkSel& pk, const uint32_t* H, const uint8_t* h_inf, const uint32_t* S,
+                         const uint8_t* s_inf, uint8_t* cls, size_t cnt, bool check_subgroup, hipStream_t st) {
   const Staging w = staging(c);
-  {
-    StageTimer tm(c, ST_MILLER, cnt, st);
-    blsk::launch_miller(pk.tab, pk.inf, pk.idx, H, h_inf, S, s_inf, cls, cnt, w.F, w.LN, std::min(cnt, kLineSub), w.FW,
-                        check_subgroup, st);
-  }
-  StageTimer tm(c, ST_FEXP, cnt, st);
-  final_exp(c, cnt, cls, st);
+  const size_t mn = serial_stages() || cnt > kLineSub ? cnt : tail_split_main(cnt, c->tail_q);
+  if (mn == cnt) {
+    {
+      StageTimer tm(c, ST_MILLER, cnt, st);
+      blsk::launch_miller(pk.tab, pk.inf, pk.idx, H, h_inf, S, s_inf, cls, cnt, w.F, w.LN, std::min(cnt, kLineSub),
+                          w.FW, check_subgroup, st);
+    }
+    StageTimer tm(c, ST_FEXP, cnt, st);
+    final_exp(c, cnt, cls, st);
+    return BLSV_OK;
+  }
+  auto mark = [&](hipStream_t s) {
+    hipEvent_t e = c->prof ? take_event(c) : nullptr;
+    if (e) (void)hipEventRecord(e, s);
+    return e;
+  };
+  auto keep = [&](ProfRec r) {
+    if (!c->prof) return;
+    if (!r.a2 || !r.b2) {
+      for (hipEvent_t e : {r.a2, r.b2})
+        if (e) c->event_pool.push_back(e);
+      r.a2 = r.b2 = nullptr;
+    }
+    if (r.a && r.b) {
+      c->recs.push_back(r);
+    } else {
+      for (hipEvent_t e : {r.a, r.b, r.a2, r.b2})
+        if (e) c->event_pool.push_back(e);
+    }
+  };
+  ProfRec rm{ST_MILLER, cnt, nullptr, nullptr}, rf{ST_FEXP, cnt, nullptr, nullptr};
+  SplitDrain drain{c};
+  const size_t rem = cnt - mn;
+  rm.a = mark(st);
+  blsk::launch_miller_lines(pk.tab, pk.inf, pk.idx, H, h_inf, S, s_inf, cls, cnt, 0, cnt, w.LN, cnt, check_subgroup, st);
+  blsk::launch_miller_f(w.LN, cnt, cls, cnt, 0, mn, w.F, w.FW, false, st);
+  rm.b = mark(st);
+  int rc = BLSV_OK;
+  auto chk = [&](hipError_t e, const char* what) {
+    if (e != hipSuccess && rc == BLSV_OK) rc = fail(c, BLSV_EHIP, "%s: %s", what, hipGetErrorString(e));
+    return e == hipSuccess;
+  };
+  if (chk(hipEventRecord(c->fork_ev, st), "split fork") && chk(hipStreamWaitEvent(c->side, c->fork_ev, 0), "split fork")) {
+    drain.armed = true;
+    rm.a2 = mark(c->side);
+    blsk::launch_miller_f(w.LN, cnt, cls, cnt, mn, rem, w.F, nullptr, true, c->side);
+    rm.b2 = mark(c->side);
+    rf.a2 = mark(c->side);
+    final_exp(c, cnt, mn, rem, cls, c->side);
+    rf.b2 = mark(c->side);
+    rf.a = mark(st);
+    final_exp(c, cnt, 0, mn, cls, st);
+    rf.b = mark(st);
+    if (chk(hipEventRecord(c->join_ev, c->side), "split join") && chk(hipStreamWaitEvent(st, c->join_ev, 0), "split join"))
+      drain.armed = false;
+  }
+  keep(rm);
+  keep(rf);
+  return rc;
 }
 
 static int finish_pass(blsv_ctx* c, size_t base, size_t cnt, const PassOut& out, hipStream_t st) {
@@ -70,8 +130,8 @@
 
 static int run_tail(blsv_ctx* c, size_t base, size_t cnt, const PkSel& pk, const PassOut& out, hipStream_t st) {
   const Staging w = staging(c);
-  pairing_check(c, pk, w.H, w.h_inf, w.S, w.s_inf, w.cls, cnt, true, st);
-  return finish_pass(c, base, cnt, out, st);
+  const int rc = pairing_check(c, pk, w.H, w.h_inf, w.S, w.s_inf, w.cls, cnt, true, st);
+  return rc ? rc : finish_pass(c, base, cnt, out, st);
 }
 
 
@@ -120,8 +180,9 @@
   int rc = rlc_sums(c, base, cnt, seed, st);
   if (rc) return rc;
   HIPCHK(c, hipMemsetAsync(r.gcls.p, 0, ng, st));
-  pairing_check(c, pk, r.gH.as<uint32_t>(), r.g_hinf.as<uint8_t>(), r.gS.as<uint32_t>(), r.g_sinf.as<uint8_t>(),
-                r.gcls.as<uint8_t>(), ng, false, st);
+  rc = pairing_check(c, pk, r.gH.as<uint32_t>(), r.g_hinf.as<uint8_t>(), r.gS.as<uint32_t>(), r.g_sinf.as<uint8_t>(),
+                     r.gcls.as<uint8_t>(), ng, false, st);
+  if (rc) return rc;
   HIPCHK(c, hipGetLastError());
   HIPCHK(c, r.host.ensure(kMaxChunk / kRlcGroupMin * 5 + 16));
   uint8_t* verdict = r.host.as<uint8_t>();
@@ -149,8 +210,9 @@
                               r.c_hinf.as<uint8_t>(), r.cS.as<uint32_t>(), r.c_sinf.as<uint8_t>(), r.ccls.as<uint8_t>(),
                               st);
     }
-    pairing_check(c, pk, r.cH.as<uint32_t>(), r.c_hinf.as<uint8_t>(), r.cS.as<uint32_t>(), r.c_sinf.as<uint8_t>(),
-                  r.ccls.as<uint8_t>(), m, false, st);
+    rc = pairing_check(c, pk, r.cH.as<uint32_t>(), r.c_hinf.as<uint8_t>(), r.cS.as<uint32_t>(), r.c_sinf.as<uint8_t>(),
+                       r.ccls.as<uint8_t>(), m, false, st);
+    if (rc) return rc;
     StageTimer tm(c, ST_RLC, m, st);
     blsk::launch_rlc_scatter(r.fail.as<uint32_t>(), G, m, r.ccls.as<uint8_t>(), w.cls, cnt, st);
   }
diff --git a/drand_amd/engine.py b/drand_amd/engine.py
--- a/drand_amd/engine.py
+++ b/drand_amd/engine.py
@@ -444,6 +444,9 @@
         self._check(self.lib.blsv_test_final_exp(self._h, Fw, n, A, B))
         return list(A)[:n * 144], list(B)[:n * 144]
 
+    def test_tail_split(self, q):
+        self._check(self.lib.blsv_test_tail_split(self._h, ctypes.c_size_t(-1).value if q is None else int(q)))
+
     def test_hash_to_g2(self, msgs):
         n = len(msgs)
         lens = (ctypes.c_uint32 * max(n, 1))(*[len(m) for m in msgs])
diff --git a/include/blsverify_testing.h b/include/blsverify_testing.h
--- a/include/blsverify_testing.h
+++ b/include/blsverify_testing.h
@@ -12,6 +12,8 @@
 int blsv_test_pairing(blsv_ctx* ctx, const uint32_t* p, const uint32_t* q, size_t n, uint32_t* out_f);
 
 int blsv_test_final_exp(blsv_ctx* ctx, const uint32_t* f, size_t n, uint32_t* out_pipeline, uint32_t* out_ref);
+
+int blsv_test_tail_split(blsv_ctx* ctx, size_t q);
 
 int blsv_test_op(blsv_ctx* ctx, const char* name, const uint32_t* in, size_t n, uint32_t* out);
 int blsv_test_op_info(int index, const char** name, int* in_fp, int* out_fp, int* lanes);
```

After: 2.447 million beacons/s (median of 6 runs). 1.5% higher.
